# snudm-starlab/VMLMF

Hardware: AMD Instinct MI355X
Metric: RNN timesteps/sec (fwd+bwd) at B=64 T=128 hid=180 r=16; 1/2/4/8 GPU (higher is better)
Workload: dtype f32; 1 GPU; BASELINE configs[1]: UCI-HAR shape, Net(MyLSTM[MyVMLMFCell]) 1 layer, B=64/GPU T=128 I=9 H=180 w_rank=16 u_rank=16, CE loss, fwd+bwd; parameters packed inside every step, as a training loop sees it (with kept parameter images: ms_per_step_kept_images); global_batch=64, batch_per_gpu=64, seq_len=128, parallelism=dp1, scaling=weak, launch=hipgraph, parameter_images=packed inside every step (what a training loop sees), criterion=vmlmf_amd.Net.loss (cross-entropy riding on the forward launch, C ABI vmlmf_ce)

## Files before the change

vmlmf_amd/csrc/vmlmf_api.hip:

```cpp
#include "vmlmf_host.h"

using namespace vmlmf_host;

namespace vmlmf_host {

int make_geo(const vmlmf_desc* d, VGeo* out, RbGeo* rbout, int force_W) {
  if (d == nullptr) return fail(VMLMF_E_BADARG, "null descriptor");
  VGeo g;
  memset(&g, 0, sizeof(g));
  g.variant = d->variant;
  g.B = d->B;
  g.T = d->T;
  g.I = d->I;
  g.H = d->H;
  g.rw = d->w_rank;
  if (d->dtype != VMLMF_DT_F32 && d->dtype != VMLMF_DT_BF16) return fail(VMLMF_E_BADARG, "dtype must be VMLMF_DT_F32 or VMLMF_DT_BF16");
  g.bf = d->dtype == VMLMF_DT_BF16 ? 1 : 0;
  if (g.variant < 1 || g.variant > 6) return fail(VMLMF_E_BADARG, "variant must be 1..6");
  if (g.B < 1 || g.T < 1 || g.I < 1 || g.H < 1 || g.rw < 1)
    return fail(VMLMF_E_BADARG, "B, T, I, H, w_rank must be positive");
  const bool grouped = g.variant == VMLMF_V2_GROUP_CELL || g.variant == VMLMF_V4_LM_GROUP ||
                       g.variant == VMLMF_V6_GROUP_NOVM;
  const bool lm = g.variant == VMLMF_V3_LM || g.variant == VMLMF_V4_LM_GROUP;
  g.novm = (g.variant == VMLMF_V5_LMF_CELL || g.variant == VMLMF_V6_GROUP_NOVM) ? 1 : 0;
  g.pergate = g.variant == VMLMF_V5_LMF_CELL ? 1 : 0;
  g.xperm = g.variant == VMLMF_V6_GROUP_NOVM ? 1 : 0;
  g.G = grouped ? d->g : 1;
  if (grouped && g.G < 1) return fail(VMLMF_E_BADARG, "g must be positive");
  if (g.G > VMLMF_MAX_G)
    return fail(VMLMF_E_UNSUPPORTED, "g > 2 is not covered by the HIP kernels (the reference never builds it)");
  if (g.H % g.G != 0) return fail(VMLMF_E_SHAPE, "hidden_size must be divisible by g (vmlmf_group.py:73)");
  if (!lm && !g.novm && g.I > g.H)
    return fail(VMLMF_E_SHAPE, "input_size > hidden_size: the reference cell raises (vmlmf.py:94,103)");

  if (lm && g.I != g.H) return fail(VMLMF_E_SHAPE, "LM layers need input_size == hidden_size (vmlmf_lm.py:243)");
  g.ru0 = d->u_ranks[0];
  g.ru1 = g.G == 2 ? d->u_ranks[1] : 0;
  if (g.ru0 < 1 || (g.G == 2 && g.ru1 < 1)) return fail(VMLMF_E_BADARG, "u_ranks must be positive");
  g.Hg = g.H / g.G;
  g.W = (g.Hg + 63) / 64;
  if (force_W > g.W) g.W = force_W;
  g.NW = g.G * g.W;
  g.NT = g.NW * 64;
  g.off1 = vg_pad8(g.ru0);
  g.KH = g.off1 + (g.G == 2 ? vg_pad8(g.ru1) : 0);
  g.KX = vg_pad8(g.rw);
  g.NP = (g.KH + 15) / 16;
  g.KQ = g.NP * 16;
  g.NPX = (g.KX + 15) / 16;
  g.KQX = g.NPX * 16;
  g.flat = g.variant == VMLMF_V4_LM_GROUP ? 1 : 0;
  g.hperm = (g.variant == VMLMF_V2_GROUP_CELL || g.variant == VMLMF_V6_GROUP_NOVM) ? 1 : 0;
  g.time_major = d->time_major ? 1 : 0;
  g.training = d->training ? 1 : 0;
  if (g.time_major) {
    g.sxT = (long long)g.B * g.I;
    g.sxB = g.I;
    g.syT = (long long)g.B * g.H;
    g.syB = g.H;
  } else {
    g.sxT = g.I;
    g.sxB = (long long)g.T * g.I;
    g.syT = g.H;
    g.syB = (long long)g.T * g.H;
  }
  g.generic = (g.KH > 32 || g.NT > 512 || g.I > g.H) ? 1 : 0;
  g.wide = (g.KX > 32 || g.G * g.KH > 128) ? 1 : 0;
  if (g.wide) {
    if (!g.generic) {
      if (g.KX > 32)
        return fail(VMLMF_E_UNSUPPORTED, "padded w_rank > 32 is not covered by the HIP kernels on a register-resident layer "
                                         "(wide ranks need the step-wise path: padded u_rank > 32, more than 512 thread slots or I > H)");
      return fail(VMLMF_E_UNSUPPORTED, "padded hidden rank (summed over groups) > 128 is not covered on a register-resident layer");
    }
    if (g.rw > g.I) return fail(VMLMF_E_UNSUPPORTED, "wide ranks: w_rank larger than input_size (an over-complete factorisation) is not covered");
    if (g.ru0 > g.Hg || (g.G == 2 && g.ru1 > g.Hg))
      return fail(VMLMF_E_UNSUPPORTED, "wide ranks: a u_rank larger than the units it factors (hidden_size / g) is not covered");
    if (g.bf) return fail(VMLMF_E_UNSUPPORTED, "wide ranks: dtype bf16 is not covered (fp32 only)");
    if (g.KX > 1024 || g.KH > 1024)
      return fail(VMLMF_E_UNSUPPORTED, "wide ranks: padded w_rank and padded hidden rank (summed over shifts) are capped at 1024, the "
                                       "bound of the step-wise workspace");
  }
  g.R = 1;
  g.nwg = (g.B + g.R - 1) / g.R;
  g.Bp = g.nwg * g.R;
  if ((long long)g.T * g.Bp * g.NT * 4 >= (1LL << 31) || (long long)g.T * g.B * g.H >= (1LL << 31))
    return fail(VMLMF_E_UNSUPPORTED, "T*B*H too large for the 32-bit element offsets of the kernels");
  const int TB = g.T * g.B;
  int rc = ((TB + 1023) / 1024 + 7) / 8 * 8;
  if (rc < 8) rc = 8;
  if (g_rc > 0) rc = g_rc;
  g.RC = rc;
  g.nblk = (TB + rc - 1) / rc;
  int rc2 = (TB + g_wchunks - 1) / g_wchunks;
  if (rc2 < g_wmin) rc2 = g_wmin;
  g.RC2 = rc2;
  g.nchunk = (TB + rc2 - 1) / rc2;
  g.foldx = (!g.generic && g.I <= g.KX) ? 1 : 0;
  g.NA = 5 * g.KX + 5 * g.KH + 12;
  {
    RbGeo q;
    memset(&q, 0, sizeof(q));
    g.rb = 0;
    if (g.bf) {
      if (!g.generic && g.I <= g.H && rb_geometry(g, 1, &q, g_rb_rows)) g.rb = 1;
      else return fail(VMLMF_E_UNSUPPORTED, "dtype bf16: implemented by the row-block MFMA kernels for one-group layers (V1, V3, V5) "
                                            "with padded rank <= 32 and <= 512 thread slots");
    } else if (g_rb_mode != 0 && g.I <= g.H && !g.wide) {
      if (g.generic) {
        const int cand[] = {g_rb_S, 16, 8, 4, 2};
        for (int i = (g_rb_S > 0 ? 0 : 1); i < 5 && g.rb == 0; ++i)
          if (cand[i] > 1 && rb_geometry(g, cand[i], &q, g_rb_rows)) g.rb = cand[i];
      } else if ((g_rb_mode == 1 || (g_rb_minB > 0 && g.B >= g_rb_minB)) && rb_geometry(g, 1, &q, g_rb_rows)) {
        g.rb = 1;
      }
    }
    if (g.rb != 0) g.foldx = 0;
    if (rbout != nullptr) *rbout = q;
  }
  {
    const long long GK = (long long)g.G * g.KH;
    const long long nb1 = (vg_nb1(g) + 31) / 32 * 32, nb2 = (GK + 31) / 32 * 32, nb3 = (g.KX + 31) / 32 * 32;
    g.PCH = (long long)g.NT * 4 * nb1 + (long long)((g.H + 31) / 32) * 32 * nb2 +
            (long long)((g.I + 31) / 32) * 32 * nb3 + 3LL * g.NT * 4;
  }
  *out = g;
  return 0;
}

static long long gemm_part_floats(const VGeo& g) { return (long long)VG_GEMM_SPLIT * ((g.B + 63) / 64 * 64) * ((g.G * g.KH + 63) / 64 * 64); }
Layout make_layout(const VGeo& g, const VPack& P, const RbGeo& q) {
  Layout L;
  const long long TB = (long long)g.T * g.B;
  const long long TS = (long long)g.T * g.Bp * g.NT;
  long long o = 0;
  L.r_pack = o, o += align64(P.total);
  const long long TBp = TB + (g.NT >= 256 ? 16 : 0);
  L.r_qx = o, o += align64(TBp * g.KX);
  L.r_gates = o, o += align64(TS * 4);
  L.r_cs = o, o += align64(TS + (long long)g.Bp * g.NT);
  L.r_Qs = o, o += align64(TBp * g.G * g.KH);
  L.r_prog = o, o += align64((long long)g.B * WR_PROG_STRIDE);
  L.r_total = o;
  o = 0;
  L.f_pack = o, o += align64(P.total);
  L.f_gx = o, o += align64(TS * 4);
  L.f_qx = o, o += align64(g.generic ? TB * g.KX : 0);
  L.f_trash = o, o += 64;
  {
    const long long gen = (g.generic && !g.rb) ? 1 : 0, BN = (long long)g.B * g.NT;
    L.f_Qtmp = o, o += align64(gen * g.B * g.G * g.KH);
    L.f_P = o, o += align64(gen * BN * 4);
    L.f_ccar = o, o += align64(gen * BN);
    L.f_zeros = o, o += align64(gen * (long long)g.B * g.H);
    L.f_part = o, o += align64(gen * gemm_part_floats(g));
  }
  L.f_xq = o, o += align64(g.rb ? q.xq_floats : 0);
  L.f_flag = o, o += align64(g.rb ? q.flag_words : 0);
  L.f_xrows = o, o += align64((g.wide && !g.time_major) ? TB * g.I : 0);
  L.f_total = o;
  o = 0;
  L.b_dpre = o, o += align64(TS * 4);
  L.b_dQs = o, o += align64(TBp * g.G * g.KH);
  L.b_dqx = o, o += align64(TBp * g.KX);
  {
    long long blocks = g.nchunk;
    if (!g.generic && !g.rb && rec4_bwd_supported(g) && g.nwg > blocks) blocks = g.nwg;
    L.b_wpart = o, o += align64(g.wide ? 0 : blocks * g.PCH);
  }
  L.b_cgrad = o, o += align64((long long)g.NA * g.NT + (g.I > g.H ? (long long)g.I * g.KX : 0));
  L.b_trash = o, o += 64;
  {
    const long long gen = (g.generic && !g.rb) ? 1 : 0, BN = (long long)g.B * g.NT;
    L.b_dHrec = o, o += align64(gen * (long long)g.B * g.H);
    L.b_ehterm = o, o += align64(gen * BN);
    L.b_dcar = o, o += align64(gen * BN);
    L.b_part = o, o += align64((g.generic ? 1 : 0) * gemm_part_floats(g));
  }
  L.b_xq = o, o += align64(g.rb ? q.xq_floats : 0);
  L.b_flag = o, o += align64(g.rb ? q.flag_words : 0);
  L.b_headdh = o, o += align64((g.rb || g.generic) ? (long long)g.B * g.H : 0);
  L.b_dux = o, o += align64((!g.generic && !g.rb && finish2_ok(g)) ? (long long)g.nchunk * (g.NT / 8) * 256 : 0);
  L.b_wide = o, o += wide_scratch_floats(g);
  L.b_total = o;
  return L;
}

template <class P>
static int check_pointers(const VGeo& g, const P* p, const char* what) {
  if (p == nullptr) return fail(VMLMF_E_BADARG, std::string("null ") + what);
  bool ok = p->u_x && p->u_h[0];
  if (g.pergate) {
    for (int k = 0; k < 4; ++k) ok = ok && p->w_gate[k] && p->u_gate[k] && p->b_gate[k];
  } else {
    ok = ok && p->v_x && p->b_x && p->b_h && p->v_h[0];
    if (!g.novm) ok = ok && p->dia_x && p->dia_h;
  }
  if (!ok) return fail(VMLMF_E_BADARG, std::string("null pointer in ") + what);
  if (g.G == 2 && (!p->u_h[1] || !p->v_h[1]))
    return fail(VMLMF_E_BADARG, std::string(what) + ": group variant needs u_h[1], v_h[1]");
  return 0;
}

int check_params(const VGeo& g, const vmlmf_params* p) { return check_pointers(g, p, "params"); }
int check_grads(const VGeo& g, const vmlmf_grads* gr) { return check_pointers(g, gr, "grads"); }
int check_head(const VGeo& g, const vmlmf_head* hd, bool fwd) {
  if (hd == nullptr || hd->classes == 0) return 0;
  if (hd->classes < 0 || hd->classes > head_max_classes()) return fail(VMLMF_E_UNSUPPORTED, "head: 1..32 classes");
  if (hd->weight == nullptr || (fwd ? hd->logits == nullptr : hd->dlogits == nullptr)) return fail(VMLMF_E_BADARG, "head: null pointer");
  return 0;
}

static void plan_wride(const VGeo& g, WRide* w) {
  const int n1 = (vg_nb1(g) + 31) / 32, n2 = (g.G * g.KH + 31) / 32;
  if (!g_wride || g_wride_tripped.load() != 0 || !g.foldx || g.flat || g.R != 1 || g.NT > 256 || g.B > g_wride_maxb || n1 > 2 || n2 > 2) return;
  const int S = (g.B % g_wride_rc == 0 && g_wride_rc % 2 == 0) ? g_wride_rc : g.B * (g.B >= 64 ? 1 : (64 + g.B - 1) / g.B);
  const int nck = (g.T * g.B + S - 1) / S;
  int K = g_wride_k < g.nchunk ? g_wride_k : g.nchunk;
  K = K < nck ? K : nck;
  const int tasks = g.NT / 8 + (g.H + 31) / 32;
  const int wpw = (g.NT + 128) / 64;
  const int ntg = (tasks + wpw - 1) / wpw;
  const int room = (device_cus() - 8 - g.nwg) / ntg;
  K = K < room ? K : room;
  if (K < 4) return;
  w->K = K, w->S = S, w->tasks = tasks, w->ntg = ntg;
  w->lag = g_wride_lag < 8 ? g_wride_lag : 8;
  w->spin = (unsigned)g_wride_spin;
}

LayerPlan plan_layer(const VGeo& g, const vmlmf_params* p, bool packed, bool head, bool want_dx, PlanCtx ctx) {
  LayerPlan pl;
  memset(&pl, 0, sizeof(pl));
  pl.family = g.rb ? FAM_RB : (g.generic ? FAM_STEP : FAM_VALU);
  pl.xwave = g_xwave && vg_xwave_ok(g);
  pl.head_inside = head && pl.family == FAM_VALU;
  pl.dqx = !(g.foldx && !want_dx);
  if (pl.family != FAM_VALU) return pl;
  const bool call = ctx == PLAN_CALL;
  if (pl.xwave && ((g_rec3 & 1) || ((g_rec3 & 4) && g.nwg > device_cus())) && rec3_fwd_supported(g)) pl.fwd = K_REC3;
  const bool rec3_bwd = (g_rec3 & 2) && rec3_bwd_supported(g);
  if (call && g_inrow != 0 && !want_dx && rec4_bwd_supported(g) && (g_inrow > 0 || g.B > g_wride_maxb)) pl.bwd = K_REC4;
  else pl.bwd = rec3_bwd ? K_REC3 : K_REC;
  if (call && pl.bwd != K_REC4) plan_wride(g, &pl.ride);
  if (pl.ride.K > 0 && pl.bwd != K_REC3 && !rec_bwd_rides(g)) memset(&pl.ride, 0, sizeof(pl.ride));
  pl.finish2 = pl.ride.K > 0 && g_finish2 != 0 && finish2_ok(g) && p->v_x != nullptr;
  const uintptr_t al = (uintptr_t)p->v_h[0] | (uintptr_t)p->u_h[0] | (uintptr_t)p->v_x | (uintptr_t)p->u_x;
  pl.direct = call && !packed && g_direct != 0 && (g.variant == VMLMF_V1_CELL || g.variant == VMLMF_V3_LM) && g.G == 1 && g.R == 1 &&
              g.foldx && pl.xwave && pl.fwd == K_REC && (g.KH == 8 || g.KH == 16) && g.ru0 == g.KH && (g.KX == 8 || g.KX == 16) &&
              g.rw == g.KX && (!g.training || rec3_bwd) && (al & 15u) == 0;
  return pl;
}

static WgxArgs wgx_args(const Layout& L, const VPack& P, const float* pack, float* ws, float* dx) {
  WgxArgs wx;
  wx.dpre = ws + L.b_dpre, wx.VRX = pack + P.VRX, wx.UXO = pack + P.UXO, wx.EXI = pack + P.EXI;
  wx.dx = dx, wx.dqx = ws + L.b_dqx;
  return wx;
}
static void split_k(GenericBuf* w, const VGeo& g, float* part, const float* pack, const VPack& P) {
  w->part = part, w->part_cap = gemm_part_floats(g);
  w->ticket = reinterpret_cast<int*>(const_cast<float*>(pack + P.TKT)), w->ticket_cap = VG_GEMM_TICKETS;
}
static void ride_buffers(LayerPlan* pl, const Layout& L, const WghArgs& wh, const vmlmf_params* p, const float* rs, float* ws, hipStream_t s) {
  WRide* w = &pl->ride;
  if (pl->bwd == K_REC4) {
    w->a.x = wh.x, w->a.y = wh.y, w->a.h0 = wh.h0, w->a.Qs = wh.Qs, w->a.P = wh.wpart;
    return;
  }
  if (w->K == 0) return;
  w->a.dpre = wh.dpre, w->a.x = wh.x, w->a.y = wh.y, w->a.h0 = wh.h0, w->a.qx = wh.qx, w->a.dqx = wh.dqx, w->a.Qs = wh.Qs;
  w->a.dQs = wh.dQs, w->a.P = wh.wpart;
  w->prog = reinterpret_cast<unsigned*>(const_cast<float*>(rs + L.r_prog));
  w->status = status_word(s);
  if (pl->finish2) w->dux = ws + L.b_dux, w->vx = p->v_x;
}

int backward_tail(const VGeo& g, const LayerPlan& pl, const Layout& L, const vmlmf_params* p, const vmlmf_grads* gr, const float* x,
                  const float* y, const float* h0, const float* rs, float* ws, const HeadBwd& hb, hipStream_t s) {
  int rc;
  const WghArgs wh = wgrad_args(L, x, y, h0, rs, ws);
  const bool rode = pl.ride.K > 0, inrow = pl.bwd == K_REC4;
  int ring_nc[3] = {0, 0, 0};
  if (g.wide) {
    const long long TB = (long long)g.T * g.B, N4 = 4LL * g.NT, GK = (long long)g.G * g.KH;
    auto al = [](long long n) { return (n + 63) / 64 * 64; };
    WideBuf wb;
    wb.x = x, wb.y = y, wb.h0 = h0, wb.dpre = wh.dpre, wb.qx = wh.qx, wb.dqx = wh.dqx, wb.Qs = wh.Qs, wb.dQs = wh.dQs;
    float* o = ws + L.b_wide;
    wb.X = o, o += al(g.time_major ? 0 : TB * g.I);
    wb.Hp = o, o += al(TB * g.H);
    wb.dVd = o, o += al(N4 * GK);
    wb.dUd = o, o += al((long long)g.H * GK);
    wb.dVx = o, o += al(N4 * g.KX);
    wb.dUx = o, o += al((long long)g.I * g.KX);
    wb.csum = o;
    wb.cgrad = ws + L.b_cgrad;
    if ((rc = run(SL_WGRAD, s, "wgrad", [&] { return wide_wgrad(g, wb, s); })) != 0) return rc;
  } else if (!rode && !inrow) {
    Scope sc(SL_WGRAD, s);
    const bool ring = g_wring != 0 && wgrad_ring_ok(g) && (g_wring > 0 || (g.generic && (long long)g.T * g.B >= 1024));
    int rr = ring ? launch_wgrad_ring(g, wh, device_cus(), ring_nc, s) : -3;
    if (rr == 0) ++g_ring_launches;
    if (rr == -3) {
      ring_nc[0] = ring_nc[1] = ring_nc[2] = 0;
      rr = launch_wgrad_h(g, wh, s);
    }
    if ((rc = hip_fail(rr, "wgrad")) != 0) return rc;
  }
  const RefG og = to_refg(gr);
  if (rode && pl.finish2)
    return run(SL_FINISH2, s, "finish2", [&] {
      return launch_finish2(g, to_refp(p), ws + L.b_wpart, pl.ride.dux, pl.ride.K, og, hb, pl.ride.prog, s, health_word(s));
    });
  if (!g.wide) {
    VGeo gr_ = g;
    if (rode) gr_.nchunk = pl.ride.K;
    if (inrow) gr_.nchunk = g.B;
    if ((rc = run(SL_REDUCE, s, "reduce", [&] {
           return launch_reduce(gr_, ws + L.b_wpart, ws + L.b_cgrad, rode ? pl.ride.prog : nullptr, s, ReduceCounts{{ring_nc[0], ring_nc[1], ring_nc[2]}});
         })) != 0) return rc;
  }
  return run(SL_FINISH, s, "finish", [&] { return launch_finish(g, to_refp(p), ws + L.b_cgrad, og, hb, s, health_word(s)); });
}

int site_drop(const vmlmf_dropout* dr, bool forward, DropArgs* out) {
  memset(out, 0, sizeof(*out));
  if (dr == nullptr) return 0;
  const int rc = drop_args(dr->p, dr->state, dr->site, forward ? dr->y_dropped : nullptr, out);
  if (rc != 0) return rc;
  if (dr->state == nullptr || (forward && dr->y_dropped == nullptr)) return fail(VMLMF_E_BADARG, "dropout: null state / y_dropped");
  return 0;
}

int valu_backward(const VGeo& g, LayerPlan* pl, const Layout& L, const VPack& P, const float* pack, const vmlmf_params* p, const LayerBwdIo& io,
                  const HeadBwd& hb, const float* rs, float* ws, hipStream_t s) {
  int rc;
  BwdArgs a;
  a.gates = rs + L.r_gates, a.cs = rs + L.r_cs, a.c0 = io.c0, a.dy = io.dy, a.dhT = io.dhT, a.dcT = io.dcT;
  a.VR = pack + P.VR, a.UE = pack + P.UE, a.EH = pack + P.EH, a.VE = pack + P.VE;
  a.dpre = ws + L.b_dpre, a.dQs = ws + L.b_dQs, a.dh0 = io.dh0, a.dc0 = io.dc0, a.trash = ws + L.b_trash;
  a.hd = hb;
  ride_buffers(pl, L, wgrad_args(L, io.x, io.y, io.h0, rs, ws), p, rs, ws, s);
  a.wr = pl->ride;
  if (pl->direct) {
    const bool own = pl->bwd == K_REC4 || pl->ride.K > 0;
    if (own) a.VE = p->v_h[0], a.UE = p->u_h[0], a.EH = p->dia_h, a.wr.direct = 1;
    if ((!own || pl->dqx) &&
        (rc = run(SL_PACK, s, "pack", [&] { return launch_pack(g, to_refp(p), P, const_cast<float*>(pack), s); })) != 0) return rc;
  }
  {
    Scope sc(SL_REC_BWD, s);
    if (pl->bwd == K_REC4) {
      if ((rc = hip_fail(launch_rec4_bwd(g, a, s), "rec4_bwd")) != 0) return rc;
    } else if (pl->bwd == K_REC3) {
      if ((rc = hip_fail(launch_rec3_bwd(g, a, s), "rec3_bwd")) != 0) return rc;
    } else if ((rc = hip_fail(launch_rec_bwd(g, a, s), "rec_bwd")) != 0) return rc;
  }
  if (!pl->dqx) return 0;
  return run(SL_DQX_DX, s, "dqx_dx", [&] { return launch_wgrad_x(g, wgx_args(L, P, pack, ws, io.dx), s); });
}

}

extern "C" {

int vmlmf_query(const vmlmf_desc* d, vmlmf_sizes* out) {
  if (out == nullptr) return fail(VMLMF_E_BADARG, "null sizes");
  VGeo g;
  RbGeo q;
  const int rc = make_geo(d, &g, &q);
  if (rc != 0) return rc;
  const VPack P = vg_pack_layout(g, q.total);
  const Layout L = make_layout(g, P, q);
  out->workspace_bytes = (size_t)L.ws_total() * sizeof(float);
  out->reserve_bytes = (size_t)L.r_total * sizeof(float);
  out->rows_per_wg = g.rb ? q.rbl : g.R;
  out->threads_per_wg = g.rb ? 256 : g.NT;
  out->workgroups = g.rb ? q.nrb * q.S : g.nwg;
  out->kx = g.KX;
  out->kh = g.KH;
  return 0;
}

constexpr int PK_HDR = 64;
struct PackSig {
  long long v[10];
  bool operator==(const PackSig& o) const { return memcmp(v, o.v, sizeof(v)) == 0; }
};
static PackSig pack_signature(const VGeo& g, const VPack& P, const RbGeo& q) {
  PackSig s;
  const long long v[10] = {g.variant, P.total, g.rb, g.generic * 2 + g.bf, g.NT, (long long)g.KH * 1000 + g.KX, q.total,
                           (long long)g.I * 100000 + g.H, (long long)g.G * 100000 + g.ru0 * 100 + g.ru1, g_tune_generation};
  memcpy(s.v, v, sizeof(v));
  return s;
}
constexpr int PK_REG = 256;
struct PackReg {
  std::mutex mu;
  const void* ptr[PK_REG] = {nullptr};
  PackSig sig[PK_REG];
  int next = 0;
  void put(const void* p, const PackSig& s) {
    std::lock_guard<std::mutex> lk(mu);
    for (int i = 0; i < PK_REG; ++i)
      if (ptr[i] == p) { sig[i] = s; return; }
    ptr[next] = p, sig[next] = s;
    next = (next + 1) % PK_REG;
  }
  int check(const void* p, const PackSig& s) {
    std::lock_guard<std::mutex> lk(mu);
    for (int i = 0; i < PK_REG; ++i)
      if (ptr[i] == p) return sig[i] == s ? 0 : 2;
    return 1;
  }
} g_packreg;
static int refuse_kept(const char* why = "") {
  return fail(VMLMF_E_UNSUPPORTED, std::string("kept parameter images: not for the step-wise / clustered layers") + why);
}
static int check_packed(const void* packed, const VGeo& g, const VPack& P, const RbGeo& q) {
  if (g.generic) return refuse_kept();
  switch (g_packreg.check(packed, pack_signature(g, P, q))) {
    case 0: return 0;
    case 1: return fail(VMLMF_E_BADARG, "packed: not an image vmlmf_pack_params made at this address (or it left the registry of the last 256 images: pack it again)");
  }
  return fail(VMLMF_E_BADARG, "packed: the image was packed for another descriptor or under another kernel selection (vmlmf_tune): pack it again");
}

int vmlmf_pack_bytes(const vmlmf_desc* d, size_t* bytes) {
  if (bytes == nullptr) return fail(VMLMF_E_BADARG, "null size");
  VGeo g;
  RbGeo q;
  const int rc = make_geo(d, &g, &q);
  if (rc != 0) return rc;
  if (g.generic) return refuse_kept(" (their image carries per-call state)");
  const VPack P = vg_pack_layout(g, q.total);
  *bytes = sizeof(float) * (size_t)(PK_HDR + P.total);
  return 0;
}

int vmlmf_pack_params(const vmlmf_desc* d, const vmlmf_params* p, void* packed, void* stream) {
  VGeo g;
  RbGeo q;
  int rc = make_geo(d, &g, &q);
  if (rc != 0) return rc;
  if ((rc = check_params(g, p)) != 0) return rc;
  if (packed == nullptr) return fail(VMLMF_E_BADARG, "null packed buffer");
  if (g.generic) return refuse_kept();
  const VPack P = vg_pack_layout(g, q.total);
  hipStream_t s = (hipStream_t)stream;
  float* img = (float*)packed + PK_HDR;
  g_packreg.put(packed, pack_signature(g, P, q));
  const RefP rp = to_refp(p);
  Scope sc(SL_PACK, s);
  if ((rc = hip_fail(launch_pack(g, rp, P, img, s), "pack")) != 0) return rc;
  if (g.rb && (rc = hip_fail(launch_rb_pack(g, q, rp, img + P.RB, s), "rb_pack")) != 0) return rc;
  return 0;
}

int vmlmf_seq_forward(const vmlmf_desc* d, const vmlmf_params* p, const float* x, const float* h0,
                      const float* c0, float* y, float* hT, float* cT, void* reserve, void* workspace,
                      size_t workspace_bytes, void* stream) {
  return vmlmf_seq_forward_packed(d, p, x, h0, c0, y, hT, cT, reserve, workspace, workspace_bytes, stream, nullptr);
}

int vmlmf_seq_forward_packed(const vmlmf_desc* d, const vmlmf_params* p, const float* x, const float* h0,
                             const float* c0, float* y, float* hT, float* cT, void* reserve, void* workspace,
                             size_t workspace_bytes, void* stream, const void* packed) {
  vmlmf_extra ex = {};
  ex.packed = packed, ex.head = nullptr, ex.ce = nullptr;
  return vmlmf_seq_forward_ex(d, p, x, h0, c0, y, hT, cT, reserve, workspace, workspace_bytes, stream, &ex);
}

static int ce_after(int B, const vmlmf_head* head, const vmlmf_ce* ce, hipStream_t s) {
  if (ce == nullptr) return 0;
  return run(SL_CE_FWD, s, "ce_fwd", [&] {
    return launch_ce_fwd(B, head->classes, head->logits, (const long long*)ce->target, (long long)ce->ignore_index, ce->loss, ce->lse,
                         ce->nvalid, ce->dlogits_unit, s);
  });
}
static int head_and_ce_after(const VGeo& g, const vmlmf_head* head, const vmlmf_ce* ce, const float* hT, hipStream_t s) {
  int rc;
  if (head != nullptr && (rc = run(SL_HEAD_FWD, s, "head_fwd", [&] {
        return launch_head_fwd(g.B, g.H, head->classes, hT, g.H, head->weight, head->bias, head->logits, s);
      })) != 0) return rc;
  return ce_after(g.B, head, ce, s);
}

static int make_drop(const vmlmf_dropout* dr, const VGeo& g, bool forward, DropArgs* out) {
  const int rc = site_drop(dr, forward, out);
  if (rc != 0 || dr == nullptr || drop_fused(g)) return rc;
  return fail(VMLMF_E_UNSUPPORTED, "dropout inside the layer's launches: row-block layers in the time-major layout (vmlmf_dropout_fused)");
}

int vmlmf_seq_forward_ex(const vmlmf_desc* d, const vmlmf_params* p, const float* x, const float* h0,
                         const float* c0, float* y, float* hT, float* cT, void* reserve, void* workspace,
                         size_t workspace_bytes, void* stream, const vmlmf_extra* ex) {
  const void* packed = ex != nullptr ? ex->packed : nullptr;
  const vmlmf_head* head = (ex != nullptr && ex->head != nullptr && ex->head->classes != 0) ? ex->head : nullptr;
  VGeo g;
  RbGeo q;
  int rc = take_status();
  if (rc != 0) return rc;
  if ((rc = make_geo(d, &g, &q)) != 0) return rc;
  if ((rc = check_params(g, p)) != 0) return rc;
  if (x == nullptr || y == nullptr || workspace == nullptr) return fail(VMLMF_E_BADARG, "null x / y / workspace");
  if (g.training && reserve == nullptr) return fail(VMLMF_E_BADARG, "training forward needs a reserve buffer");
  if ((rc = check_head(g, head, true)) != 0) return rc;
  const LayerPlan pl = plan_layer(g, p, packed != nullptr, head != nullptr, true);
  if (head != nullptr && !pl.head_inside && hT == nullptr) return fail(VMLMF_E_BADARG, "head on this layer needs the hT output");
  DropArgs drop;
  if ((rc = make_drop(ex != nullptr ? ex->drop : nullptr, g, true, &drop)) != 0) return rc;
  const vmlmf_ce* ce = ex != nullptr ? ex->ce : nullptr;
  if (ce != nullptr) {
    if (head == nullptr) return fail(VMLMF_E_BADARG, "ce: the criterion rides on the classifier's logits (extra.head)");
    if (!ce->target || !ce->loss || !ce->nvalid || !ce->lse || !ce->ticket) return fail(VMLMF_E_BADARG, "ce: null pointer");
  }
  const VPack P = vg_pack_layout(g, q.total);
  const Layout L = make_layout(g, P, q);
  if (workspace_bytes < (size_t)L.ws_total() * sizeof(float))
    return fail(VMLMF_E_WORKSPACE, "workspace smaller than vmlmf_query() reported");
  hipStream_t s = (hipStream_t)stream;
  float* ws = (float*)workspace;
  float* rs = (float*)reserve;
  float* pack = g.training ? rs + L.r_pack : ws + L.f_pack;
  if (packed != nullptr) {
    if ((rc = check_packed(packed, g, P, q)) != 0) return rc;
    pack = const_cast<float*>((const float*)packed) + PK_HDR;
  }
  float* gx = ws + L.f_gx;
  const RefP rp = to_refp(p);
  if (packed == nullptr && !pl.direct && (rc = run(SL_PACK, s, "pack", [&] { return launch_pack(g, rp, P, pack, s); })) != 0) return rc;
  float* const qxbuf = g.training ? rs + L.r_qx : (g.generic ? ws + L.f_qx : nullptr);
  if (!pl.xwave && (rc = run(SL_XPROJ, s, "xproj", [&] {
        return g.wide ? wide_xproj(g, P, pack, x, ws + L.f_xrows, gx, qxbuf, s) : launch_xproj(g, P, pack, x, gx, qxbuf, s);
      })) != 0) return rc;
  if (pl.family == FAM_RB) {
    if (packed == nullptr && (rc = run(SL_PACK, s, "rb_pack", [&] {
          return launch_rb_pack(g, q, rp, pack + P.RB, s, reinterpret_cast<unsigned*>(ws + L.f_flag));
        })) != 0) return rc;
    RbIo io;
    memset(&io, 0, sizeof(io));
    io.flags_zeroed = packed == nullptr ? 1 : 0;
    io.gx = gx, io.EH = pack + P.EH, io.h0 = h0, io.c0 = c0, io.img = pack + P.RB, io.y = y, io.hT = hT, io.cT = cT;
    io.gates = g.training ? rs + L.r_gates : nullptr, io.cs = g.training ? rs + L.r_cs : nullptr;
    io.Qs = g.training ? rs + L.r_Qs : nullptr;
    io.xq = ws + L.f_xq, io.flag = reinterpret_cast<unsigned*>(ws + L.f_flag), io.status = status_word(s);
    io.drop = drop;
    if ((rc = run(SL_REC_FWD, s, "rb_fwd", [&] { return launch_rb_fwd(g, q, io, s); })) != 0) return rc;
    return head_and_ce_after(g, head, ce, hT, s);
  }
  if (pl.family == FAM_STEP) {
    GenericBuf w;
    memset(&w, 0, sizeof(w));
    w.gx = gx, w.EH = pack + P.EH, w.h0 = h0, w.c0 = c0, w.Ud = pack + P.UD, w.Vd = pack + P.VD;
    w.UdT = pack + P.UDT;
    w.zeros = ws + L.f_zeros, w.y = y, w.hT = hT, w.cT = cT;
    w.gates = g.training ? rs + L.r_gates : nullptr, w.cs = g.training ? rs + L.r_cs : nullptr;
    w.Qs = g.training ? rs + L.r_Qs : nullptr, w.Qtmp = ws + L.f_Qtmp, w.P = ws + L.f_P, w.ccar = ws + L.f_ccar;
    split_k(&w, g, ws + L.f_part, pack, P);
    if (h0 == nullptr) {
      rc = (int)hipMemsetAsync(ws + L.f_zeros, 0, sizeof(float) * (size_t)g.B * g.H, s);
      if (rc != 0) return hip_fail(rc, "memset");
    }
    if ((rc = run(SL_REC_FWD, s, "generic_forward", [&] { return generic_forward(g, w, s); })) != 0) return rc;
    return head_and_ce_after(g, head, ce, hT, s);
  }
  FwdArgs a;
  a.gx = gx, a.VE = pack + P.VE, a.UR = pack + P.UR, a.EH = pack + P.EH, a.h0 = h0, a.c0 = c0;
  a.y = y, a.hT = hT, a.cT = cT, a.trash = ws + L.f_trash;
  a.gates = g.training ? rs + L.r_gates : nullptr;
  a.cs = g.training ? rs + L.r_cs : nullptr;
  a.Qs = g.training ? rs + L.r_Qs : nullptr;
  XwArgs xw;
  xw.x = x, xw.UXP = pack + P.UXP, xw.WXD = pack + P.WXD, xw.BBT = pack + P.BBT;
  memset(&xw.hd, 0, sizeof(xw.hd));
  if (pl.head_inside) xw.hd.W = head->weight, xw.hd.bias = head->bias, xw.hd.logits = head->logits, xw.hd.C = head->classes;
  memset(&xw.ce, 0, sizeof(xw.ce));
  if (pl.head_inside && ce != nullptr && g.R == 1 && g.B < 65536) {
    xw.ce.tgt = (const long long*)ce->target, xw.ce.ignore = (long long)ce->ignore_index, xw.ce.loss = ce->loss, xw.ce.nvalid = ce->nvalid;
    xw.ce.lse = ce->lse, xw.ce.dz = ce->dlogits_unit, xw.ce.ticket = (unsigned long long*)ce->ticket;
  }
  a.xwave = pl.xwave ? 1 : 0, a.qxw = g.training ? rs + L.r_qx : nullptr;
  xw.BH = nullptr, xw.DX = nullptr, xw.direct = 0, xw.pad = 0;
  if (pl.direct) {
    a.VE = p->v_h[0], a.UR = p->u_h[0], a.EH = p->dia_h, a.xwave = 3;
    xw.UXP = p->u_x, xw.WXD = p->v_x, xw.BBT = p->b_x, xw.BH = p->b_h, xw.DX = p->dia_x, xw.direct = 1;
  }
  a.prog = g.training ? reinterpret_cast<unsigned*>(rs + L.r_prog) : nullptr;
  if ((rc = pl.fwd == K_REC3 ? run(SL_REC_FWD, s, "rec3_fwd", [&] { return launch_rec3_fwd(g, a, xw, s); })
                             : run(SL_REC_FWD, s, "rec_fwd", [&] { return launch_rec_fwd(g, a, xw, s); })) != 0) return rc;
  if (ce != nullptr && xw.ce.tgt == nullptr && (rc = ce_after(g.B, head, ce, s)) != 0) return rc;
  return debug_status(s);
}

int vmlmf_seq_backward(const vmlmf_desc* d, const vmlmf_params* p, const float* x, const float* h0,
                       const float* c0, const float* y, const void* reserve, const float* dy,
                       const float* dhT, const float* dcT, float* dx, float* dh0, float* dc0,
                       const vmlmf_grads* gr, void* workspace, size_t workspace_bytes, void* stream) {
  return vmlmf_seq_backward_packed(d, p, x, h0, c0, y, reserve, dy, dhT, dcT, dx, dh0, dc0, gr, workspace, workspace_bytes, stream,
                                   nullptr);
}

int vmlmf_seq_backward_packed(const vmlmf_desc* d, const vmlmf_params* p, const float* x, const float* h0,
                              const float* c0, const float* y, const void* reserve, const float* dy,
                              const float* dhT, const float* dcT, float* dx, float* dh0, float* dc0,
                              const vmlmf_grads* gr, void* workspace, size_t workspace_bytes, void* stream,
                              const void* packed) {
  vmlmf_extra ex = {};
  ex.packed = packed, ex.head = nullptr, ex.ce = nullptr;
  return vmlmf_seq_backward_ex(d, p, x, h0, c0, y, reserve, dy, dhT, dcT, dx, dh0, dc0, gr, workspace, workspace_bytes, stream, &ex);
}

int vmlmf_seq_backward_ex(const vmlmf_desc* d, const vmlmf_params* p, const float* x, const float* h0,
                          const float* c0, const float* y, const void* reserve, const float* dy,
                          const float* dhT, const float* dcT, float* dx, float* dh0, float* dc0,
                          const vmlmf_grads* gr, void* workspace, size_t workspace_bytes, void* stream,
                          const vmlmf_extra* ex) {
  const void* packed = ex != nullptr ? ex->packed : nullptr;
  const vmlmf_head* head = (ex != nullptr && ex->head != nullptr && ex->head->classes != 0) ? ex->head : nullptr;
  VGeo g;
  RbGeo q;
  int rc = take_status();
  if (rc != 0) return rc;
  if ((rc = make_geo(d, &g, &q)) != 0) return rc;
  if ((rc = check_params(g, p)) != 0) return rc;
  if (x == nullptr || y == nullptr || reserve == nullptr || workspace == nullptr || gr == nullptr)
    return fail(VMLMF_E_BADARG, "null x / y / reserve / workspace / grads");
  if ((rc = check_grads(g, gr)) != 0) return rc;
  if ((rc = check_head(g, head, false)) != 0) return rc;
  LayerPlan pl = plan_layer(g, p, packed != nullptr, head != nullptr, dx != nullptr);
  DropArgs drop;
  if ((rc = make_drop(ex != nullptr ? ex->drop : nullptr, g, false, &drop)) != 0) return rc;
  const VPack P = vg_pack_layout(g, q.total);
  const Layout L = make_layout(g, P, q);
  if (workspace_bytes < (size_t)L.ws_total() * sizeof(float))
    return fail(VMLMF_E_WORKSPACE, "workspace smaller than vmlmf_query() reported");
  hipStream_t s = (hipStream_t)stream;
  float* ws = (float*)workspace;
  const float* rs = (const float*)reserve;
  const float* hlast = y + (size_t)(g.T - 1) * g.syT;
  const HeadBwd hb = head_bwd_args(pl.head_inside ? head : nullptr, g, y);
  if (head != nullptr && !pl.head_inside) {
    if (dhT != nullptr) return fail(VMLMF_E_UNSUPPORTED, "head together with an explicit dhT: only on the VALU recurrent kernels");
    float* tmp = ws + L.b_headdh;
    if ((rc = run(SL_HEAD_BWD, s, "head_bwd", [&] {
           return launch_head_bwd(g.B, g.H, head->classes, hlast, g.syB, head->weight, head->dlogits, tmp, head->dweight, head->dbias, s);
         })) != 0) return rc;
    dhT = tmp;
  }
  const float* pack = rs + L.r_pack;
  if (packed != nullptr) {
    if ((rc = check_packed(packed, g, P, q)) != 0) return rc;
    pack = (const float*)packed + PK_HDR;
  }
  if (pl.family == FAM_RB) {
    RbIo io;
    memset(&io, 0, sizeof(io));
    io.gates = const_cast<float*>(rs + L.r_gates), io.cs = const_cast<float*>(rs + L.r_cs), io.EH = pack + P.EH;
    io.img = pack + P.RB, io.dy = dy, io.dhT = dhT, io.dcT = dcT, io.dpre = ws + L.b_dpre, io.dQs = ws + L.b_dQs;
    io.dh0 = dh0, io.dc0 = dc0, io.xq = ws + L.b_xq, io.flag = reinterpret_cast<unsigned*>(ws + L.b_flag), io.status = status_word(s);
    io.drop = drop;
    if ((rc = run(SL_REC_BWD, s, "rb_bwd", [&] { return launch_rb_bwd(g, q, io, s); })) != 0) return rc;
    if (g.generic) {
      GenericBuf w;
      memset(&w, 0, sizeof(w));
      w.dpre = ws + L.b_dpre, w.VxT = pack + P.VXTT, w.dqx = ws + L.b_dqx, w.dx = dx, w.UXP = pack + P.UXP, w.EXT = pack + P.EXT;
      split_k(&w, g, ws + L.b_part, pack, P);
      if ((rc = run(SL_DQX_DX, s, "dqx_dx", [&] { return generic_dqx_dx(g, w, s); })) != 0) return rc;
    } else if ((rc = run(SL_DQX_DX, s, "dqx_dx", [&] { return launch_wgrad_x(g, wgx_args(L, P, pack, ws, dx), s); })) != 0) {
      return rc;
    }
  } else if (pl.family == FAM_STEP) {
    GenericBuf w;
    memset(&w, 0, sizeof(w));
    w.EH = pack + P.EH, w.gates = const_cast<float*>(rs + L.r_gates), w.cs = const_cast<float*>(rs + L.r_cs);
    w.dy = dy, w.dhT = dhT, w.dcT = dcT, w.UdT = pack + P.UDT, w.VdT = pack + P.VDT, w.VxT = pack + P.VXTT;
    w.UXP = pack + P.UXP, w.EXT = pack + P.EXT, w.Vd = pack + P.VD;
    w.dpre = ws + L.b_dpre, w.dQs = ws + L.b_dQs, w.dHrec = ws + L.b_dHrec, w.ehterm = ws + L.b_ehterm;
    w.dcar = ws + L.b_dcar, w.dh0 = dh0, w.dc0 = dc0, w.dqx = ws + L.b_dqx, w.dx = dx;
    if (g.wide) {
      w.UXT = pack + P.UXT;
      w.dxs = ws + L.b_total - ((long long)g.T * g.B * g.I + 63) / 64 * 64;
    }
    split_k(&w, g, ws + L.b_part, pack, P);
    if ((rc = run(SL_REC_BWD, s, "generic_backward", [&] { return generic_backward(g, w, s); })) != 0) return rc;
  } else if ((rc = valu_backward(g, &pl, L, P, pack, p, LayerBwdIo{x, y, h0, c0, dy, dhT, dcT, dx, dh0, dc0}, hb, rs, ws, s)) != 0) {
    return rc;
  }
  if ((rc = backward_tail(g, pl, L, p, gr, x, y, h0, rs, ws, hb, s)) != 0) return rc;
  return debug_status(s);
}

}
```

vmlmf_amd/csrc/vmlmf_host.h:

```cpp
#pragma once
#include <hip/hip_runtime.h>

#include <atomic>
#include <cstdio>
#include <cstring>
#include <mutex>
#include <string>
#include <vector>

#include "../../include/vmlmf_hip.h"
#include "vmlmf_launch.h"

#pragma GCC visibility push(hidden)
namespace vmlmf_host {

int fail(int code, const std::string& msg);
int hip_fail(int rc, const char* what);
inline int hip_tail(int rc) { return rc == 0 ? 0 : fail(rc, hipGetErrorString((hipError_t)rc)); }

extern int g_debug_sync, g_adam_guard, g_xwave, g_wchunks, g_wmin, g_rc, g_wride, g_wride_k, g_wride_maxb, g_wride_lag, g_wride_rc, g_rb_mode,
    g_rb_minB, g_rb_S, g_rb_rows, g_rec3, g_inrow, g_wring, g_direct, g_finish2, g_wf_bwd, g_pack_slim, g_finish_units, g_rbx, g_ffb;
extern int g_wride_spin, g_tune_generation;
extern std::atomic<int> g_wride_tripped;
extern std::atomic<int> g_ring_launches;

enum Slot { SL_PACK, SL_XPROJ, SL_REC_FWD, SL_REC_BWD, SL_DQX_DX, SL_WGRAD, SL_REDUCE, SL_FINISH, SL_HEAD_FWD, SL_HEAD_BWD, SL_CE_FWD,
            SL_CE_BWD, SL_FINISH2, NKERN };
inline const char* kernel_label(int k) {
  static const char* const names[NKERN] = {"pack_kernel",     "xproj_kernel",      "rec_fwd_kernel",   "rec_bwd_kernel",
                                           "dqx_dx_kernel",   "wgrad_mfma_kernel", "reduce_cg_kernel", "finish_kernel",
                                           "head_fwd_kernel", "head_bwd_kernel",   "ce_fwd_kernel",    "ce_bwd_kernel", "finish2_kernel"};
  return (k >= 0 && k < NKERN) ? names[k] : "";
}
struct Prof {
  std::mutex mu;
  unsigned mask = 0;
  std::vector<std::pair<hipEvent_t, hipEvent_t>> ev[NKERN];
};
extern Prof g_prof;

struct Scope {
  int k;
  hipStream_t s;
  hipEvent_t e0 = nullptr, e1 = nullptr;
  Scope(Slot which, hipStream_t st) : k(which), s(st) {
    if (g_debug_sync) fprintf(stderr, "[vmlmf] launching %s\n", kernel_label(which));
    if ((g_prof.mask >> which) & 1u) {
      (void)hipEventCreate(&e0);
      (void)hipEventCreate(&e1);
      (void)hipEventRecord(e0, s);
    }
  }
  ~Scope() {
    if (g_debug_sync) {
      const hipError_t e = hipStreamSynchronize(s);
      fprintf(stderr, "[vmlmf] %s done: %s\n", kernel_label(k), hipGetErrorString(e));
    }
    if (e0 != nullptr) {
      (void)hipEventRecord(e1, s);
      std::lock_guard<std::mutex> lk(g_prof.mu);
      g_prof.ev[k].push_back({e0, e1});
    }
  }
};
template <class F>
int run(Slot k, hipStream_t s, const char* what, F&& launch) {
  Scope sc(k, s);
  return hip_fail((int)launch(), what);
}

unsigned* status_word(hipStream_t s);
unsigned* health_word(hipStream_t s);
int take_status();
int debug_status(hipStream_t s);
int device_cus();

inline long long align64(long long v) { return (v + 63) / 64 * 64; }
int make_geo(const vmlmf_desc* d, VGeo* out, RbGeo* rbout = nullptr, int force_W = 0);
struct Layout {
  long long r_pack, r_qx, r_gates, r_cs, r_Qs, r_prog, r_total;
  long long f_pack, f_gx, f_qx, f_trash, f_Qtmp, f_P, f_ccar, f_zeros, f_part, f_xq, f_flag, f_xrows, f_total;
  long long b_dpre, b_dQs, b_dqx, b_wpart, b_cgrad, b_trash, b_dHrec, b_ehterm, b_dcar, b_part, b_xq, b_flag, b_headdh, b_dux, b_wide, b_total;
  long long ws_total() const { return f_total > b_total ? f_total : b_total; }
};
Layout make_layout(const VGeo& g, const VPack& P, const RbGeo& q);

inline RefP to_refp(const vmlmf_params* p) {
  RefP r;
  r.dia_x = p->dia_x, r.dia_h = p->dia_h, r.u_x = p->u_x, r.v_x = p->v_x, r.b_x = p->b_x, r.b_h = p->b_h;
  r.u_h0 = p->u_h[0], r.u_h1 = p->u_h[1], r.v_h0 = p->v_h[0], r.v_h1 = p->v_h[1];
  for (int k = 0; k < 4; ++k) r.wg[k] = p->w_gate[k], r.ug[k] = p->u_gate[k], r.bg[k] = p->b_gate[k];
  return r;
}
inline RefG to_refg(const vmlmf_grads* gr) {
  RefG og;
  og.dia_x = gr->dia_x, og.dia_h = gr->dia_h, og.u_x = gr->u_x, og.v_x = gr->v_x, og.b_x = gr->b_x;
  og.b_h = gr->b_h, og.u_h0 = gr->u_h[0], og.u_h1 = gr->u_h[1], og.v_h0 = gr->v_h[0], og.v_h1 = gr->v_h[1];
  for (int k = 0; k < 4; ++k) og.wg[k] = gr->w_gate[k], og.ug[k] = gr->u_gate[k], og.bg[k] = gr->b_gate[k];
  return og;
}

int check_params(const VGeo& g, const vmlmf_params* p);
int check_grads(const VGeo& g, const vmlmf_grads* gr);
int check_head(const VGeo& g, const vmlmf_head* hd, bool fwd);

inline int drop_args(float p, const void* state, int site, float* yd, DropArgs* out) {
  memset(out, 0, sizeof(*out));
  if (!(p >= 0.f && p < 1.f)) return fail(VMLMF_E_BADARG, "dropout: p must be in [0, 1)");
  out->state = reinterpret_cast<const unsigned long long*>(state), out->yd = yd;
  out->thresh = drop_thresh(p), out->scale = 1.f / (1.f - p), out->site = site;
  return 0;
}
int site_drop(const vmlmf_dropout* dr, bool forward, DropArgs* out);
inline bool drop_fused(const VGeo& g) { return g.rb && g.syT == (long long)g.B * g.H; }

enum Family { FAM_RB, FAM_STEP, FAM_VALU };
enum RecKernel { K_REC, K_REC3, K_REC4 };
enum PlanCtx { PLAN_CALL, PLAN_CHAINED };
struct LayerPlan {
  Family family;
  bool xwave;
  RecKernel fwd, bwd;
  bool direct;
  bool head_inside;
  bool dqx;
  bool finish2;
  WRide ride;
};
LayerPlan plan_layer(const VGeo& g, const vmlmf_params* p, bool packed, bool head, bool want_dx, PlanCtx ctx = PLAN_CALL);

inline WghArgs wgrad_args(const Layout& L, const float* x, const float* y, const float* h0, const float* rs, float* ws) {
  WghArgs wh;
  wh.dpre = ws + L.b_dpre, wh.x = x, wh.y = y, wh.h0 = h0, wh.qx = rs + L.r_qx, wh.dqx = ws + L.b_dqx;
  wh.Qs = rs + L.r_Qs, wh.dQs = ws + L.b_dQs, wh.wpart = ws + L.b_wpart;
  return wh;
}
inline HeadBwd head_bwd_args(const vmlmf_head* head, const VGeo& g, const float* y) {
  HeadBwd hb;
  memset(&hb, 0, sizeof(hb));
  if (head == nullptr) return hb;
  hb.W = head->weight, hb.dl = head->dlogits, hb.hlast = y + (size_t)(g.T - 1) * g.syT, hb.ldh = g.syB, hb.dW = head->dweight, hb.db = head->dbias;
  hb.C = head->classes;
  return hb;
}
struct LayerBwdIo {
  const float *x, *y, *h0, *c0, *dy, *dhT, *dcT;
  float *dx, *dh0, *dc0;
};
int valu_backward(const VGeo& g, LayerPlan* pl, const Layout& L, const VPack& P, const float* pack, const vmlmf_params* p, const LayerBwdIo& io,
                  const HeadBwd& hb, const float* rs, float* ws, hipStream_t s);
int backward_tail(const VGeo& g, const LayerPlan& pl, const Layout& L, const vmlmf_params* p, const vmlmf_grads* gr, const float* x,
                  const float* y, const float* h0, const float* rs, float* ws, const HeadBwd& hb, hipStream_t s);

}
#pragma GCC visibility pop
```

vmlmf_amd/csrc/vmlmf_launch.h:

```cpp
#pragma once
#include <hip/hip_runtime.h>
#include "vmlmf_device.h"
#include "vmlmf_dropout.h"

#define VG_REC_BOUNDS (MAXT + 128)

enum EnvRule { ENV_SET, ENV_ON, ENV_INT, ENV_POS };
int vmlmf_env_switch(const char* name, EnvRule rule, int dflt);

struct HeadFwd {
  const float *W, *bias;
  float* logits;
  int C, pad;
};
struct HeadBwd {
  const float *W, *dl;
  const float* hlast;
  float *dW, *db;
  long long ldh;
  int C, pad;
};

struct FwdArgs {
  const float *gx, *VE, *UR, *EH, *h0, *c0;
  float *y, *hT, *cT, *gates, *cs, *Qs;
  float* trash;
  float* qxw;
  int xwave;
  unsigned* prog;
};
struct CeFwd {
  const long long* tgt;
  long long ignore;
  float *loss, *nvalid;
  float *lse, *dz;
  unsigned long long* ticket;
};
struct XwArgs {
  const float *x, *UXP, *WXD, *BBT;
  HeadFwd hd;
  CeFwd ce;
  const float *BH, *DX;
  int direct, pad;
};
struct AtbArgs {
  const float *dpre, *x, *y, *h0, *qx, *dqx, *Qs, *dQs;
  float* P;
  int pad0, pad;
};
constexpr int WR_PROG_STRIDE = 32;
constexpr unsigned VMLMF_ST_WRIDE = 1, VMLMF_ST_CLUSTER = 2, VMLMF_ST_WF_FWD = 3, VMLMF_ST_WF_BWD = 4, VMLMF_ST_P2P = 5;
__device__ __forceinline__ void vg_raise(unsigned* status, unsigned code) {
  if (status != nullptr) __hip_atomic_store(status, code, __ATOMIC_RELAXED, __HIP_MEMORY_SCOPE_SYSTEM);
}
struct WRide {
  AtbArgs a;
  float* dux;
  const float* vx;
  unsigned* prog;
  int K, S, ntg, tasks;
  int lag;
  int direct;
  unsigned spin;
  unsigned* status;
};
struct BwdArgs {
  const float *gates, *cs, *c0, *dy, *dhT, *dcT, *VR, *UE, *EH;
  const float* VE;
  float *dpre, *dQs, *dh0, *dc0;
  float* trash;
  HeadBwd hd;
  WRide wr;
};
struct WgxArgs {
  const float *dpre, *VRX, *UXO, *EXI;
  float *dx, *dqx;
};
struct WghArgs {
  const float *dpre, *x, *y, *h0, *qx, *dqx, *Qs, *dQs;
  float* wpart;
};

struct GenericBuf {
  const float *gx, *EH, *h0, *c0, *Ud, *Vd, *zeros;
  float *y, *hT, *cT, *gates, *cs, *Qs, *Qtmp, *P, *ccar;
  const float *dy, *dhT, *dcT, *UdT, *VdT, *VxT, *UXP, *EXT;
  float *dpre, *dQs, *dHrec, *ehterm, *dcar, *dh0, *dc0, *dqx, *dx;
  const float* UXT;
  float* dxs;
  float* part;
  long long part_cap;
  int* ticket;
  int ticket_cap;
};
int generic_forward(const VGeo& g, const GenericBuf& w, hipStream_t s);
int generic_backward(const VGeo& g, const GenericBuf& w, hipStream_t s);
int generic_dqx_dx(const VGeo& g, const GenericBuf& w, hipStream_t s);
int generic_qx(const VGeo& g, const float* x, const float* UXP, float* qx, hipStream_t s);
int wide_xproj(const VGeo& g, const VPack& L, const float* pack, const float* x, float* xrows, float* gx, float* qx, hipStream_t s);
constexpr int WIDE_NCH = 64;
struct WideBuf {
  const float *x, *y, *h0, *dpre, *qx, *dqx, *Qs, *dQs;
  float *X, *Hp;
  float *dVd, *dUd, *dVx, *dUx;
  float *csum;
  float *cgrad;
};
inline long long wide_scratch_floats(const VGeo& g) {
  if (!g.wide) return 0;
  const long long TB = (long long)g.T * g.B, N4 = 4LL * g.NT, GK = (long long)g.G * g.KH;
  auto al = [](long long n) { return (n + 63) / 64 * 64; };
  return al(g.time_major ? 0 : TB * g.I) + al(TB * g.H) + al(N4 * GK) + al((long long)g.H * GK) + al(N4 * g.KX) +
         al((long long)g.I * g.KX) + al((long long)WIDE_NCH * 3 * N4) + al(TB * g.I);
}
int wide_wgrad(const VGeo& g, const WideBuf& w, hipStream_t s);

constexpr int RBX_MAXL = 4;
struct RbIo {
  const float *gx, *EH, *h0, *c0, *img, *dy, *dhT, *dcT;
  float *y, *hT, *cT, *gates, *cs, *Qs, *dpre, *dQs, *dh0, *dc0;
  float* xq;
  unsigned* flag;
  unsigned* status;
  int flags_zeroed;
  DropArgs drop;
};
bool rb_geometry(const VGeo& g, int S, RbGeo* out, int rows = 0, int xf = 0);

struct RbxLayerF {
  const float *x, *EH, *EXT, *BBT, *h0, *c0, *img;
  float *y, *hT, *cT, *gates, *cs, *Qs, *qx;
  float* xq;
  unsigned* flag;
  const unsigned* pflag;
  int pub, pad;
  DropArgs drop;
};
struct RbxLayerB {
  const float *gates, *cs, *dy, *dhT, *dcT, *EH, *EXT, *img;
  float *dpre, *dQs, *dqx, *dx, *dh0, *dc0;
  float* xq;
  unsigned* flag;
  const unsigned* pflag;
  int pub, pad;
  DropArgs drop;
};
struct RbxFwdArgs {
  unsigned* status;
  int L, bpl;
  RbxLayerF l[RBX_MAXL];
};
struct RbxBwdArgs {
  unsigned* status;
  int L, bpl;
  RbxLayerB l[RBX_MAXL];
};
struct RbxZeroArgs {
  float* dpre[RBX_MAXL];
  unsigned* flags[RBX_MAXL];
};
bool rbx_supported(const VGeo& g, const RbGeo& q);
int launch_rbx_fwd(const VGeo& g, const RbGeo& q, const RbxFwdArgs& a, hipStream_t s);
int launch_rbx_bwd(const VGeo& g, const RbGeo& q, const RbxBwdArgs& a, hipStream_t s);
int launch_rbx_zero(const VGeo& g, const RbGeo& q, int L, float* const* dpre, unsigned* const* flags, hipStream_t s);
int launch_rb_pack(const VGeo& g, const RbGeo& q, const RefP& p, float* img, hipStream_t s, unsigned* zero_flags = nullptr);
int launch_rb_fwd(const VGeo& g, const RbGeo& q, const RbIo& io, hipStream_t s);
int launch_rb_pack_stack(const VGeo& g, const RbGeo& q, int L, const RefP* p, float* const* img, unsigned* const* zero_flags, hipStream_t s);
int launch_rb_bwd(const VGeo& g, const RbGeo& q, const RbIo& io, hipStream_t s);

int launch_pack(const VGeo& g, const RefP& p, const VPack& L, float* pack, hipStream_t s);
int launch_xproj(const VGeo& g, const VPack& L, const float* pack, const float* x, float* gx, float* qx,
                 hipStream_t s);
int launch_rec_fwd(const VGeo& g, const FwdArgs& a, const XwArgs& xw, hipStream_t s);
int launch_rec_bwd(const VGeo& g, const BwdArgs& a, hipStream_t s);
inline bool rec_bwd_rides(const VGeo& g) { return g.KH > 16 || g.W > 3; }
bool rec3_fwd_supported(const VGeo& g);
bool rec3_bwd_supported(const VGeo& g);
int launch_rec3_fwd(const VGeo& g, const FwdArgs& a, const XwArgs& xw, hipStream_t s);
int launch_rec3_bwd(const VGeo& g, const BwdArgs& a, hipStream_t s);
bool rec4_bwd_supported(const VGeo& g);
int launch_rec4_bwd(const VGeo& g, const BwdArgs& a, hipStream_t s);
int launch_wgrad_x(const VGeo& g, const WgxArgs& a, hipStream_t s);
int launch_wgrad_h(const VGeo& g, const WghArgs& a, hipStream_t s);
bool wgrad_ring_ok(const VGeo& g);
int launch_wgrad_ring(const VGeo& g, const WghArgs& a, int cus, int nc_out[3], hipStream_t s);
struct ReduceCounts {
  int c[3];
};
int launch_reduce(const VGeo& g, const float* wpart, float* cgrad, unsigned* prog, hipStream_t s,
                  ReduceCounts wc = ReduceCounts{{0, 0, 0}});
bool finish2_ok(const VGeo& g);
int launch_finish2(const VGeo& g, const RefP& p, const float* wpart, const float* dux, int K, const RefG& out, const HeadBwd& hd,
                   unsigned* prog, hipStream_t s, unsigned* health);
int launch_finish(const VGeo& g, const RefP& p, const float* cgrad, const RefG& out, const HeadBwd& hd, hipStream_t s,
                  unsigned* health = nullptr);
unsigned* vmlmf_health_word_if_any();
int vmlmf_adam_guard_mode();

int head_max_classes();
hipError_t launch_head_fwd(int B, int H, int C, const float* h, long long ldh, const float* W, const float* bias,
                           float* out, hipStream_t s);
hipError_t launch_head_bwd(int B, int H, int C, const float* h, long long ldh, const float* W, const float* dl,
                           float* dh, float* dW, float* db, hipStream_t s);

hipError_t launch_ce_fwd(int B, int C, const float* z, const long long* tgt, long long ignore_index, float* loss,
                         float* lse, float* nvalid, float* dz_unit, hipStream_t s);
hipError_t launch_ce_bwd(int B, int C, const float* z, const long long* tgt, long long ignore_index,
                         const float* lse, const float* nvalid, const float* dloss, float* dz, hipStream_t s);

hipError_t launch_nll_fwd(int R, int V, const float* scores, const long long* y, float scale, float* loss, float* lse,
                          float* rowloss, hipStream_t s);
hipError_t launch_nll_bwd(int R, int V, const float* scores, const long long* y, float scale, const float* lse,
                          const float* dloss, float* dscores, hipStream_t s);

int head_loss_workgroups(int R);
int launch_nll_fwd_grad(int R, int V, float* scores, const float* bias, const long long* y, float scale, float* loss,
                        float* rowloss, float* dbias, float* scratch, hipStream_t s);
int launch_distill_fwd_grad(int R, int V, float* scores, const float* bias, const long long* y, float scale, float alpha, float tau,
                            const float* teacher, const long long* top_tokens, const float* top_scores, int top, float* loss,
                            float* rowloss, float* dbias, float* scratch, hipStream_t s);
struct ObjectiveArgs {
  float eps, zeta, alpha;
  const long long* negatives;
  int k;
  const float* scale_dev;
};
int launch_objective_fwd_grad(int R, int V, float* scores, const float* bias, const long long* y, float scale, const ObjectiveArgs& o,
                              float* loss, float* rowloss, float* dbias, float* scratch, hipStream_t s);
size_t embed_bwd_scratch_bytes(int R, int V);
int launch_transpose(int rows, int cols, const float* src, float* dst, hipStream_t s);
int launch_embed_bwd(int R, int H, int V, const long long* tokens, const float* dy, float* dW, void* scratch, size_t scratch_bytes,
                     hipStream_t s, const DropArgs* drop = nullptr);
int launch_drop_advance(unsigned long long* state, unsigned long long* snap, hipStream_t s);
int launch_drop_rows(int mode, long long R, int H, int V, const DropArgs& d, const DropCols& cm, const float* x, const long long* tokens, float* y,
                     hipStream_t s);
struct LmSampleArgs {
  const float *h, *w, *bias, *embed;
  const unsigned long long* state;
  long long* tokens;
  float *logprob, *x_next;
  float* part;
  unsigned long long* ticket;
  float inv_temp;
  int B, H, V, step, tpw;
  int top_k;
  float top_p;
  int* kept;
  float* scores;
};
size_t lm_sample_workspace_bytes(int B, int V);
size_t lm_sample_filtered_workspace_bytes(int B, int V);
int launch_lm_sample(LmSampleArgs a, hipStream_t s);
struct LmChooseArgs {
  const float *scores, *bias, *embed;
  const unsigned long long* state;
  long long* tokens;
  float *logprob, *x_next;
  float inv_temp;
  int B, H, V, step;
  int top_k;
  float top_p;
  int* kept;
};
int launch_lm_choose(const LmChooseArgs& a, hipStream_t s);

constexpr int WF_MAXL = 4;
constexpr int WF_FLAG_STRIDE = 32;
struct WfPack {
  long long UR, VR, URX, VRX;
  long long VE, UE, VXK, UXK;
  long long total;
};
__host__ __device__ inline int wf_width(const VGeo& g) { return g.KH > g.KX ? g.KH : g.KX; }
struct WfFwdLayer {
  const float* x;
  const float *VE, *EH, *VXT, *EXT, *BBT;
  const float *UR, *URX;
  const float *h0, *c0;
  float *y, *hT, *cT, *gates, *cs, *Qs, *qx;
  long long sxT, sxB;
  long long syT, syB;
  int I, H;
  int Hg, pad;
};
struct WfBwdLayer {
  const float *gates, *cs, *dy, *dhT, *dcT;
  const float *UE, *EH, *UXO, *EXI;
  const float *VR, *VRX;
  float *dpre, *dQs, *dqx, *dx, *dh0, *dc0;
  long long sxT, sxB;
  long long syT, syB;
  int I, want_dx;
  int H, Hg;
};
struct WfCommon {
  unsigned* flag;
  unsigned* status;
  int L, pad;
};
struct WfFwdArgs {
  WfCommon c;
  WfFwdLayer l[WF_MAXL];
  HeadFwd hd;
  DropArgs drop[WF_MAXL];
};
struct WfBwdArgs {
  WfCommon c;
  WfBwdLayer l[WF_MAXL];
  HeadBwd hd;
  DropArgs drop[WF_MAXL];
};
bool wf_supported(const VGeo& g);
WfPack wf_pack_layout(const VGeo& g);
int launch_pack_stack(int L, const VGeo* g, const RefP* p, const VPack* P, const WfPack& W, float* const* pack, unsigned* zero0,
                      int nzero0, unsigned* zero1, int nzero1, hipStream_t s, int images = 0);
enum { PACK_ALL = 0, PACK_CLUSTERED = 1, PACK_WAVEFRONT = 2 };
int launch_wf_fwd(const VGeo& g, const WfFwdArgs& a, hipStream_t s);
int launch_wf_bwd(const VGeo& g, const WfBwdArgs& a, hipStream_t s);
int launch_wgrad_h_stack(int L, const VGeo* g, const WghArgs* w, hipStream_t s);
struct AtbStack;
int launch_wgrad4_stack(int L, const VGeo* g, const WghArgs* w, const AtbStack& S, hipStream_t s);
int wgrad4_chunk_rows(int L, const VGeo* g, int cus);
int launch_reduce_stack(int L, const VGeo* g, const float* const* wpart, float* const* cgrad, hipStream_t s,
                        const ReduceCounts* wc = nullptr);
bool finish_from_blocks_ok(const VGeo& g);
int launch_finish_stack(int L, const VGeo* g, const RefP* p, const float* const* cgrad, const RefG* out, const HeadBwd& hd_top,
                        hipStream_t s, unsigned* health = nullptr, const float* const* wpart = nullptr,
                        const ReduceCounts* wc = nullptr);
bool finish_units_ok(const VGeo& g);
int launch_finish_units_stack(int L, const VGeo* g, const RefP* p, const RefG* out, const HeadBwd& hd_top, hipStream_t s,
                              unsigned* health, const float* const* wpart, const ReduceCounts* wc);

bool rec_supported(const VGeo& g);
```

vmlmf_amd/csrc/vmlmf_rec_fwd.inc:

```
#include "vmlmf_launch.h"
#include "vmlmf_direct.inc"

constexpr int FWD_NB = 6;


template <typename S>
__device__ __forceinline__ void copy_from_kernarg(S* dst, const __attribute__((address_space(4))) char* src) {
  static_assert(sizeof(S) % 4 == 0, "dword-sized argument structs");
  const __attribute__((address_space(4))) int* w = (const __attribute__((address_space(4))) int*)src;
  int tmp[sizeof(S) / 4];
#pragma unroll
  for (unsigned i = 0; i < sizeof(S) / 4; ++i) tmp[i] = w[i];
  __builtin_memcpy(dst, tmp, sizeof(S));
}
constexpr size_t karg_align8(size_t v) { return (v + 7) & ~(size_t)7; }
constexpr size_t KARG_FWD = karg_align8(sizeof(VGeo));
constexpr size_t KARG_XW = karg_align8(KARG_FWD + sizeof(FwdArgs));

__device__ __forceinline__ float wave_total(float v) {
  v = add_ror16<8>(v);
  v = add_ror16<4>(v);
  v = add_ror16<2>(v);
  v = add_ror16<1>(v);
  return rowsum4(v);
}
__device__ __forceinline__ float wave_max64(float v) {
#pragma unroll
  for (int o = 32; o >= 1; o >>= 1) v = fmaxf(v, __shfl_xor(v, o, 64));
  return v;
}
__device__ __attribute__((noinline)) void head_epilogue(const __attribute__((address_space(4))) char* ka,
                                                        const __attribute__((address_space(3))) float* ch, int row, int wave,
                                                        __attribute__((address_space(3))) float* lscr) {
  if (((const __attribute__((address_space(4))) int*)(ka + KARG_XW + offsetof(XwArgs, hd) + offsetof(HeadFwd, C)))[0] <= 0) return;
  VGeo g;
  XwArgs xa;
  copy_from_kernarg(&g, ka);
  copy_from_kernarg(&xa, ka + KARG_XW);
  const HeadFwd hd = xa.hd;
  if (hd.C <= 0 || row >= g.B) return;
  const int lane = threadIdx.x & 63, H = g.H, NT = g.NT, C = hd.C, NW = g.NW;
  constexpr int CP = 8;
  for (int c0 = wave; c0 < C; c0 += CP * NW) {
    float acc[CP];
#pragma unroll
    for (int j = 0; j < CP; ++j) acc[j] = 0.f;
    for (int slot = lane; slot < NT; slot += 64) {
      int n;
      const bool valid = vg_slot_unit(g, slot, n);
      const float hv = valid ? ch[slot * 2 + 1] : 0.f;
      const int nc = valid ? n : 0;
      float w[CP];
#pragma unroll
      for (int j = 0; j < CP; ++j) w[j] = hd.W[(size_t)(c0 + j * NW < C ? c0 + j * NW : 0) * H + nc];
#pragma unroll
      for (int j = 0; j < CP; ++j) acc[j] = fmaf(hv, c0 + j * NW < C ? w[j] : 0.f, acc[j]);
    }
#pragma unroll
    for (int j = 0; j < CP; ++j) {
      const float t = wave_total(acc[j]);
      const int c = c0 + j * NW;
      if (lane == 0 && c < C) {
        const float z = t + (hd.bias != nullptr ? hd.bias[c] : 0.f);
        hd.logits[(size_t)row * C + c] = z;
        lscr[c] = z;
      }
    }
  }
}

__device__ __attribute__((noinline)) void ce_epilogue(const __attribute__((address_space(4))) char* ka, int row, int wave,
                                                      __attribute__((address_space(3))) float* lscr) {
  if (((const __attribute__((address_space(4))) long long*)(ka + KARG_XW + offsetof(XwArgs, ce) + offsetof(CeFwd, tgt)))[0] == 0) return;
  VGeo g;
  XwArgs xa;
  copy_from_kernarg(&g, ka);
  copy_from_kernarg(&xa, ka + KARG_XW);
  const CeFwd ce = xa.ce;
  const int lane = threadIdx.x & 63, C = xa.hd.C, B = g.B;
  if (C <= 0 || row >= B) return;
  asm volatile("s_waitcnt lgkmcnt(0)\n\ts_barrier" ::: "memory");
  if (wave != 0) return;
  const float z = lane < C ? lscr[lane] : -INFINITY;
  const float m = wave_max64(z);
  const float l = m + logf(wave_total(lane < C ? expf(z - m) : 0.f));
  int cnt = 0;
  for (int b = lane; b < B; b += 64) cnt += ce.tgt[b] != ce.ignore ? 1 : 0;
#pragma unroll
  for (int o = 32; o >= 1; o >>= 1) cnt += __shfl_xor(cnt, o, 64);
  const float nv = (float)cnt, scale = 1.f / nv;
  const long long t = ce.tgt[row];
  const bool counted = t != ce.ignore, inr = t >= 0 && t < C;
  const float rl = counted ? (inr ? l - lscr[inr ? (int)t : 0] : NAN) : 0.f;
  if (ce.dz != nullptr && lane < C) ce.dz[(size_t)row * C + lane] = counted ? scale * (expf(z - l) - (lane == (int)t ? 1.f : 0.f)) : 0.f;
  typedef unsigned long long u64;
  int lb = 0;
  while ((1 << lb) < B) ++lb;
  const int SH = 35 - lb;
  const bool fits = rl >= 0.f && rl < 2048.f;
  u64 mine = (u64)1 << 48, old = 0;
  if (fits) mine += (u64)__double2ll_rn((double)rl * (double)((u64)1 << SH));
  if (lane == 0) {
    ce.lse[row] = l;
    if (!fits) {
      const bool nan = rl != rl, big = !nan && !(rl < (float)((u64)1 << (36 - lb)));
      const u64 add1 = nan ? (u64)1 << 63 : (big ? (u64)1 << 62 : (u64)__double2ll_rn((double)rl * 1024.0));
      u64 r1;
      if (nan || big) r1 = __hip_atomic_fetch_or(ce.ticket + 1, add1, __ATOMIC_RELAXED, __HIP_MEMORY_SCOPE_AGENT);
      else r1 = __hip_atomic_fetch_add(ce.ticket + 1, add1, __ATOMIC_RELAXED, __HIP_MEMORY_SCOPE_AGENT);
      asm volatile("" :: "v"(r1) : "memory");
      __hip_atomic_fetch_or(ce.ticket, (u64)1 << 47, __ATOMIC_RELAXED, __HIP_MEMORY_SCOPE_AGENT);
    }
    old = __hip_atomic_fetch_add(ce.ticket, mine, __ATOMIC_RELAXED, __HIP_MEMORY_SCOPE_AGENT);
  }
  const unsigned olo = __builtin_amdgcn_readfirstlane((unsigned)old), ohi = __builtin_amdgcn_readfirstlane((unsigned)(old >> 32));
  const u64 total = (((u64)ohi << 32) | olo) + mine, flag = total & ((u64)1 << 47);
  if ((unsigned)(total >> 48) != (unsigned)B) return;
  double sum = (double)(total & (((u64)1 << 47) - 1)) / (double)((u64)1 << SH);
  if (flag != 0) {
    const u64 w1 = __hip_atomic_load(ce.ticket + 1, __ATOMIC_RELAXED, __HIP_MEMORY_SCOPE_AGENT);
    sum += (double)(w1 & (((u64)1 << 47) - 1)) / 1024.0;
    if ((w1 >> 62) & 1) sum = (double)INFINITY;
    if ((w1 >> 63) & 1) sum = (double)NAN;
  }
  if (lane == 0) {
    ce.loss[0] = (float)(sum / (double)nv);
    ce.nvalid[0] = nv;
    __hip_atomic_store(ce.ticket, (u64)0, __ATOMIC_RELAXED, __HIP_MEMORY_SCOPE_AGENT);
    if (flag != 0) __hip_atomic_store(ce.ticket + 1, (u64)0, __ATOMIC_RELAXED, __HIP_MEMORY_SCOPE_AGENT);
  }
}

constexpr int XW_SLOTS = 3;
constexpr int XW_NB = 12;
constexpr int XW_DIST = 8;

__host__ __device__ inline size_t xwave_lds_floats() { return (size_t)XW_NB * 64 + 2 * 32; }

template <int IM, int IE = IM>
__device__ __attribute__((noinline)) void xwave_role(const __attribute__((address_space(4))) char* ka, float* gxs,
                                                     float* xlds, int row, int ring_nb) {
  VGeo g;
  XwArgs xa;
  copy_from_kernarg(&g, ka);
  copy_from_kernarg(&xa, ka + KARG_XW);
  const int lane = threadIdx.x & 63;
  const int I = g.I, H = g.H, NT = g.NT, T = g.T, KX = g.KX;
  typedef __attribute__((address_space(3))) float lds_f;
  typedef __attribute__((address_space(3))) f32x4 lds_f4;
  lds_f* xring = (lds_f*)xlds;
  lds_f* qxs = xring + XW_NB * 64;
  lds_f* gxl = (lds_f*)gxs;
  const bool rowok = row < g.B;
  const int rowc = rowok ? row : g.B - 1;

  f32x2 w01[XW_SLOTS][IM], w23[XW_SLOTS][IM], b01[XW_SLOTS], b23[XW_SLOTS];
  float uxc[IM];
  bool real[XW_SLOTS];
  if (xa.direct != 0) {
    asm volatile("s_waitcnt lgkmcnt(0)\n\ts_barrier" ::: "memory");
    const lds_f* wxl = (const lds_f*)xlds + xwave_lds_floats();
#pragma unroll
    for (int i = 0; i < XW_SLOTS; ++i) {
      const int slot = lane + 64 * i;
      real[i] = slot < NT;
      const int sc = real[i] ? slot : 0;
#pragma unroll
      for (int m = 0; m < IM; ++m) {
        const bool mk = real[i] && m < I;
        const int mc = m < I ? m : 0;
        const float q0 = wxl[(mc * 4 + 0) * NT + sc], q1 = wxl[(mc * 4 + 1) * NT + sc];
        const float q2 = wxl[(mc * 4 + 2) * NT + sc], q3 = wxl[(mc * 4 + 3) * NT + sc];
        w01[i][m] = mk ? f32x2{q0, q1} : f32x2{0.f, 0.f};
        w23[i][m] = mk ? f32x2{q2, q3} : f32x2{0.f, 0.f};
      }
      const float c0 = wxl[(4 * I + 0) * NT + sc], c1 = wxl[(4 * I + 1) * NT + sc], c2 = wxl[(4 * I + 2) * NT + sc], c3 = wxl[(4 * I + 3) * NT + sc];
      b01[i] = real[i] ? f32x2{c0, c1} : f32x2{0.f, 0.f};
      b23[i] = real[i] ? f32x2{c2, c3} : f32x2{0.f, 0.f};
    }
  } else
#pragma unroll
  for (int i = 0; i < XW_SLOTS; ++i) {
    const int slot = lane + 64 * i;
    int n = 0;
    real[i] = slot < NT;
    const bool valid = real[i] && vg_slot_unit(g, slot, n);
    const int sc = real[i] ? slot : 0, nc = valid ? n : 0;
#pragma unroll
    for (int m = 0; m < IM; ++m) {
      const bool mk = valid && m < I;
      const int mc = m < I ? m : 0;
      w01[i][m] = mk ? f32x2{xa.WXD[(size_t)(mc * 4 + 0) * NT + sc], xa.WXD[(size_t)(mc * 4 + 1) * NT + sc]} : f32x2{0.f, 0.f};
      w23[i][m] = mk ? f32x2{xa.WXD[(size_t)(mc * 4 + 2) * NT + sc], xa.WXD[(size_t)(mc * 4 + 3) * NT + sc]} : f32x2{0.f, 0.f};
    }
    b01[i] = valid ? f32x2{xa.BBT[0 * H + nc], xa.BBT[1 * H + nc]} : f32x2{0.f, 0.f};
    b23[i] = valid ? f32x2{xa.BBT[2 * H + nc], xa.BBT[3 * H + nc]} : f32x2{0.f, 0.f};
  }
#pragma unroll
  for (int m = 0; m < IM; ++m) uxc[m] = (m < I && lane < KX && g.foldx == 0) ? xa.UXP[(m < I ? m : 0) * KX + (lane < KX ? lane : 0)] : 0.f;

  const float* xrow = xa.x + ((size_t)rowc * g.sxB + (lane < I ? lane : 0));
  size_t xoff = 0;
  auto issue = [&](int ttarget) {
    __builtin_amdgcn_global_load_lds((gl_cvoid_t*)(xrow + xoff), (lds_void_t*)(xring + (ttarget % XW_NB) * 64), 4, 0, 0);
    if (ttarget + 1 < T) xoff += (size_t)g.sxT;
  };
  auto produce = [&](int t) {
    float sx[IM];
    const lds_f4* xr4 = (const lds_f4*)(xring + (t % XW_NB) * 64);
#pragma unroll
    for (int m4 = 0; m4 < IM / 4; ++m4) {
      const f32x4 v = xr4[m4];
      sx[4 * m4 + 0] = (rowok && 4 * m4 + 0 < I) ? v[0] : 0.f;
      sx[4 * m4 + 1] = (rowok && 4 * m4 + 1 < I) ? v[1] : 0.f;
      sx[4 * m4 + 2] = (rowok && 4 * m4 + 2 < I) ? v[2] : 0.f;
      sx[4 * m4 + 3] = (rowok && 4 * m4 + 3 < I) ? v[3] : 0.f;
    }
    float q = 0.f;
    if (g.foldx == 0) {
#pragma unroll
      for (int m = 0; m < IM; ++m) q = fmaf(sx[m], uxc[m], q);
    }
    if (g.foldx == 0 && lane < KX) qxs[(t & 1) * 32 + lane] = q;
    lds_f* dst = gxl + (size_t)(t % ring_nb) * NT * 4;
#pragma unroll
    for (int i = 0; i < XW_SLOTS; ++i) {
      if (real[i]) {
        f32x2 p01a = b01[i], p01b = f32x2{0.f, 0.f}, p23a = b23[i], p23b = f32x2{0.f, 0.f};
#pragma unroll
        for (int m = 0; m + 1 < IE; m += 2) {
          p01a = pk_fma(splat2(sx[m]), w01[i][m], p01a);
          p23a = pk_fma(splat2(sx[m]), w23[i][m], p23a);
          p01b = pk_fma(splat2(sx[m + 1]), w01[i][m + 1], p01b);
          p23b = pk_fma(splat2(sx[m + 1]), w23[i][m + 1], p23b);
        }
        if constexpr ((IE & 1) != 0) {
          p01a = pk_fma(splat2(sx[IE - 1]), w01[i][IE - 1], p01a);
          p23a = pk_fma(splat2(sx[IE - 1]), w23[i][IE - 1], p23a);
        }
        const f32x2 p01 = p01a + p01b, p23 = p23a + p23b;
        *(lds_f4*)(dst + (size_t)(lane + 64 * i) * 4) = f32x4{p01.x, p01.y, p23.x, p23.y};
      }
    }
  };
  for (int s0 = 0; s0 < XW_DIST; ++s0) issue(s0);
  asm volatile("s_waitcnt vmcnt(%0)" ::"n"(XW_DIST - 1) : "memory");
  produce(0);
  wait_vm_barrier<XW_DIST - 2>();
  for (int t = 0; t < T; ++t) {
    issue(t + XW_DIST);
    produce(t + 1);
    wait_vm_barrier<XW_DIST - 2>();
  }
}

template <int KH, int R, bool FLAT, int MAXT, int CNT, bool XW = false>
__global__ void __launch_bounds__(VG_REC_BOUNDS) rec_fwd_kernel(VGeo g, FwdArgs a, XwArgs xwargs) {
  constexpr int NP = (KH + 15) / 16, KQ = NP * 16, NC = KH / 4;
  const int tid = threadIdx.x, lane = tid & 63, wave = tid >> 6;
  const int NT = g.NT, NW = g.NW, W = g.W, H = g.H, B = g.B, T = g.T;
  const bool mover = tid >= NT;
  const bool train = a.gates != nullptr;
  const size_t sstride = (size_t)g.Bp * NT;

  extern __shared__ float4 smem4[];
  float* part = reinterpret_cast<float*>(smem4);
  float* gxs = part + 2 * R * NW * KQ;
  float* outs = gxs + FWD_NB * R * NT * 4;
  float* zero4 = outs + 2 * R * NT * 8 + 256;
  if (tid < 4) zero4[tid] = 0.f;

  if (mover) {
    constexpr int MAXS = MAXT / 64;
    constexpr int NDMA = R * MAXS;
    constexpr int DEPTH = (2 * NDMA <= 63) ? 2 : 1;
    constexpr int DIST = DEPTH + 2;
    static_assert(DIST < FWD_NB, "gx ring too shallow");
    float* spare = outs + 2 * R * NT * 8;
    int row[R];
    bool rok[R];
#pragma unroll
    for (int r = 0; r < R; ++r) {
      row[r] = blockIdx.x * R + r;
      rok[r] = row[r] < B;
    }
    if (wave == NW) {
      if constexpr (XW) {
        const __attribute__((address_space(4))) char* ka =
            (const __attribute__((address_space(4))) char*)__builtin_amdgcn_kernarg_segment_ptr();
        float* xlds = zero4 + 4;
        switch ((g.I + 3) / 4) {
          case 1: xwave_role<4>(ka, gxs, xlds, row[0], FWD_NB); break;
          case 2: xwave_role<8>(ka, gxs, xlds, row[0], FWD_NB); break;
          case 3:
            if (g.I == 9) xwave_role<12, 9>(ka, gxs, xlds, row[0], FWD_NB);
            else if (g.I == 10) xwave_role<12, 10>(ka, gxs, xlds, row[0], FWD_NB);
            else xwave_role<12>(ka, gxs, xlds, row[0], FWD_NB);
            break;
          default: xwave_role<16>(ka, gxs, xlds, row[0], FWD_NB); break;
        }
        return;
      }
      auto issue = [&](int ttarget) {
        const int tc = ttarget < T ? ttarget : T - 1;
        float* dst = gxs + (size_t)(ttarget % FWD_NB) * R * NT * 4;
#pragma unroll
        for (int r = 0; r < R; ++r)
#pragma unroll
          for (int i = 0; i < MAXS; ++i) {
            const bool real = i < NW;
            const int i0 = real ? i : 0;
            dma16(a.gx + ((size_t)tc * sstride + (size_t)row[r] * NT + lane + 64 * i0) * 4,
                  real ? dst + ((size_t)r * NT + 64 * i0) * 4 : spare);
          }
      };
      for (int s0 = 0; s0 < DIST; ++s0) issue(s0);
      wait_vm_barrier<(DIST - 2) * NDMA>();
      for (int t = 0; t < T; ++t) {
        issue(t + DIST);
        wait_vm_barrier<DEPTH * NDMA>();
      }
      return;
    }
    __builtin_amdgcn_s_setprio(3);
    if (a.prog != nullptr && lane < R && rok[lane < R ? lane : 0])
      a.prog[(size_t)(blockIdx.x * R + lane) * WR_PROG_STRIDE] = 0u;
    bool sv[R][MAXS];
    unsigned so_[R][MAXS], yo_[R][MAXS];
#pragma unroll
    for (int r = 0; r < R; ++r)
#pragma unroll
      for (int i = 0; i < MAXS; ++i) {
        const int slot = lane + 64 * (i < NW ? i : 0);
        int n;
        const bool valid = vg_slot_unit(g, slot, n);
        sv[r][i] = i < NW && valid && rok[r];
        so_[r][i] = (unsigned)(row[r] * NT + slot) * 4u;
        yo_[r][i] = (unsigned)((rok[r] ? row[r] : 0) * g.syB + n) * 4u;
      }
    constexpr int QE = 2;
    bool qv[QE];
    unsigned qsrc[QE], qdst[QE];
#pragma unroll
    for (int q = 0; q < QE; ++q) {
      const int e = lane + 64 * q;
      const int GK = g.G * KH;
      const bool in = e < R * GK;
      const int ec = in ? e : 0;
      const int r = ec / GK, jr = ec - r * GK, j = jr / KH, rr = jr - j * KH;
      const int s = (g.G == 2 && rr >= g.off1) ? 1 : 0;
      const int w0 = ((j + s) % g.G) * W;
      qv[q] = in && train && (blockIdx.x * R + r) < B;
      qsrc[q] = (unsigned)((r * NW + w0) * KQ + rr);
      qdst[q] = (unsigned)((blockIdx.x * R + r) * GK + jr);
    }
    const float* qxs = zero4 + 4 + XW_NB * 64;
    const bool qx_out = XW && train && g.foldx == 0 && rok[0] && lane < g.KX;
    constexpr bool SAFE_ST = FLAT && MAXT == 512;
    auto segment = [&](int td, int tq) {
      __builtin_amdgcn_s_setprio(3);
      const int tdc = td < 0 ? 0 : td, tqc = tq < 0 ? 0 : tq;
      const float* src = outs + (size_t)(tdc & 1) * R * NT * 8;
      const float* qsrc_ = part + (size_t)(tqc & 1) * R * NW * KQ;
      float4 g4[R][MAXS];
      float2 ch[R][MAXS];
      float v[QE][MAXS];
      float qxv = 0.f;
#pragma unroll
      for (int r = 0; r < R; ++r)
#pragma unroll
        for (int i = 0; i < MAXS; ++i) {
          const int slot = lane + 64 * (i < NW ? i : 0);
          g4[r][i] = ld4(src + ((size_t)r * NT + slot) * 4);
          ch[r][i] = *reinterpret_cast<const float2*>(src + (size_t)R * NT * 4 + ((size_t)r * NT + slot) * 2);
        }
#pragma unroll
      for (int q = 0; q < QE; ++q)
#pragma unroll
        for (int w = 0; w < MAXS; ++w) v[q][w] = qsrc_[qsrc[q] + (w < W ? w : 0) * KQ];
      if constexpr (XW) qxv = qxs[(tqc & 1) * 32 + (lane & 31)];
      __builtin_amdgcn_s_setprio(0);
      if (td >= 0) {
        char* gt = reinterpret_cast<char*>(a.gates + (size_t)td * sstride * 4);
        char* ct = reinterpret_cast<char*>(a.cs + (size_t)(td + 1) * sstride);
        char* yt = reinterpret_cast<char*>(a.y + (size_t)td * g.syT);
#pragma unroll
        for (int r = 0; r < R; ++r) {
#pragma unroll
          for (int i = 0; i < MAXS; ++i) {
            if (i < NW) {
              if (train) {
                st4_sv<SAFE_ST, !SAFE_ST>(gt, 4u * so_[r][i], g4[r][i]);
                st1_sv<SAFE_ST, !SAFE_ST>(ct, so_[r][i], ch[r][i].x);
              }
              if (sv[r][i]) st1_sv<SAFE_ST, !SAFE_ST>(yt, yo_[r][i], ch[r][i].y);
            }
          }
        }
      }
      if (tq >= 0) {
        const float* qt = a.Qs + (size_t)tq * B * g.G * KH;
#pragma unroll
        for (int q = 0; q < QE; ++q) {
          if (qv[q]) {
            float acc = 0.f;
#pragma unroll
            for (int w = 0; w < MAXS; ++w) acc += w < W ? v[q][w] : 0.f;
            st1_sv<SAFE_ST>(qt, 4u * qdst[q], acc);
          }
        }
        if constexpr (XW) {
          if (qx_out) st1_sv<SAFE_ST>(a.qxw + (size_t)tq * B * g.KX, 4u * (unsigned)(row[0] * g.KX + lane), qxv);
        }
      }
    };
    if constexpr (XW) {
      if ((a.xwave & 2) != 0) asm volatile("s_barrier" ::: "memory");
    }
    asm volatile("s_waitcnt lgkmcnt(0)\n\ts_barrier" ::: "memory");
    for (int t = 0; t < T; ++t) {
      segment(t - 1, t);
      asm volatile("s_waitcnt lgkmcnt(0)\n\ts_barrier" ::: "memory");
    }
    segment(T - 1, -1);
    return;
  }

  const int grp = tid / (64 * W);
  const int m = tid - grp * 64 * W;
  const bool valid = m < g.Hg;
  const int n = grp * g.Hg + (valid ? m : 0);

  f32x2 ve01[KH], ve23[KH], eh01, eh23;
  float ur[KQ];
  bool direct = false;
  constexpr bool CAN_DIRECT = XW && KH <= 16 && !FLAT && R == 1;
  if constexpr (CAN_DIRECT) direct = (a.xwave & 2) != 0;
  if (direct) {
    if constexpr (CAN_DIRECT) {
      float vr[4][16], ur0[16], bs[4];
#pragma unroll
      for (int k = 0; k < 4; ++k) dr_load_row<KH>(a.VE, (size_t)k * H + n, valid, vr[k]);
      dr_load_row<KH>(a.UR, (size_t)n, valid, ur0);
      {
        float bxv[4], bhv[4];
#pragma unroll
        for (int k = 0; k < 4; ++k) bxv[k] = xwargs.BBT[(size_t)k * H + n], bhv[k] = xwargs.BH[(size_t)k * H + n];
#pragma unroll
        for (int k = 0; k < 4; ++k) bs[k] = bxv[k] + bhv[k];
      }
      const float dh = a.EH[n], dxv = xwargs.DX[n < g.I ? n : 0];
      const float vf = valid ? 1.f : 0.f;
      float* wxl = zero4 + 4 + xwave_lds_floats();
      auto xside = [&](auto kxc) {
        constexpr int KX_ = decltype(kxc)::value;
        float vx[4][16];
#pragma unroll
        for (int k = 0; k < 4; ++k) dr_load_row<KX_>(xwargs.WXD, (size_t)k * H + n, valid, vx[k]);
        dr_wx_unit<KX_>(vx, bs, dxv, xwargs.UXP, g.I, NT, n, vf, tid, wxl);
      };
      if (g.KX == 16) xside(std::integral_constant<int, 16>{});
      else xside(std::integral_constant<int, 8>{});
      __builtin_amdgcn_sched_barrier(0);
#pragma unroll
      for (int rr = 0; rr < KH; ++rr) ve01[rr] = f32x2{vr[0][rr], vr[1][rr]}, ve23[rr] = f32x2{vr[2][rr], vr[3][rr]};
      eh01 = f32x2{(dh - dr_chain<KH>(ur0, vr[0])) * vf, (dh - dr_chain<KH>(ur0, vr[1])) * vf};
      eh23 = f32x2{(dh - dr_chain<KH>(ur0, vr[2])) * vf, (dh - dr_chain<KH>(ur0, vr[3])) * vf};
      float* scr = outs + (size_t)tid * DR_SCR_FLOATS;
      dr_put(scr, ur0);
      const int li = lane & 15, dn = 16 - dr_ror_dir(lane);
      sfor<16>([&](auto kk) {
        constexpr int K = decltype(kk)::value;
        ur[K] = ror16<K>(dr_at(scr, li + dn * K));
      });
      asm volatile("s_waitcnt lgkmcnt(0)\n\ts_barrier" ::: "memory");
    }
  } else {
#pragma unroll
    for (int rr = 0; rr < KH; ++rr) {
      ve01[rr] = f32x2{a.VE[(size_t)(0 * KH + rr) * NT + tid], a.VE[(size_t)(1 * KH + rr) * NT + tid]};
      ve23[rr] = f32x2{a.VE[(size_t)(2 * KH + rr) * NT + tid], a.VE[(size_t)(3 * KH + rr) * NT + tid]};
    }
    eh01 = f32x2{a.EH[0 * NT + tid], a.EH[1 * NT + tid]};
    eh23 = f32x2{a.EH[2 * NT + tid], a.EH[3 * NT + tid]};
#pragma unroll
    for (int j = 0; j < KQ; ++j) ur[j] = a.UR[(size_t)j * NT + tid];
  }

  int pb[NC];
  int pb2[FLAT ? NC : 1];
#pragma unroll
  for (int c = 0; c < NC; ++c) {
    const int s = (g.G == 2 && 4 * c >= g.off1) ? 1 : 0;
    const int q0 = FLAT ? 0 : grp;
    pb[c] = (((q0 + s) % g.G) * W) * KQ + 4 * c;
    if (FLAT) pb2[c] = (((1 + s) % g.G) * W) * KQ + 4 * c;
  }

  constexpr int NCP = NC <= 2 ? 2 : (NC <= 4 ? 4 : 8);
  constexpr bool FASTQ16 = !FLAT && NC == NCP && NC * CNT <= 16;
  constexpr bool FASTQ64 = !FLAT && !FASTQ16 && NC <= 8 && NCP * CNT <= 64;
  constexpr bool FLATQ = FLAT && NC <= 8 && NCP * CNT <= 32;
  constexpr bool FASTQ = FASTQ16 || FASTQ64 || FLATQ;
  int rdoff = 0;
  {
    const int li = FLATQ ? (lane & 31) : (FASTQ64 ? lane : (lane & 15)), cc = li % NCP, w = li / NCP;
    const int ccl = cc < NC ? cc : 0;
    const int s = (g.G == 2 && 4 * ccl >= g.off1) ? 1 : 0;
    const int q0 = FLATQ ? (lane >> 5) : grp;
    rdoff = (w < CNT && cc < NC) ? ((((q0 + s) % g.G) * W + w) * KQ + 4 * cc) : -1;
  }

  float h[R], c[R];
#pragma unroll
  for (int r = 0; r < R; ++r) {
    const int row = blockIdx.x * R + r;
    const bool ok = valid && row < B;
    const int rowc = row < B ? row : B - 1;
    h[r] = (ok && a.h0 != nullptr) ? a.h0[(size_t)rowc * H + n] : 0.f;
    c[r] = (ok && a.c0 != nullptr) ? a.c0[(size_t)rowc * H + n] : 0.f;
    if (train) a.cs[(size_t)row * NT + tid] = c[r];
  }

  for (int t = 0; t < T; ++t) {
    const int buf = t & 1;
#pragma unroll
    for (int r = 0; r < R; ++r) {
      float hv = h[r];
      dpp_fence(hv);
#pragma unroll
      for (int p = 0; p < NP; ++p) {
        float a0 = 0.f, a1 = 0.f;
        fmac_ror_x16(a0, a1, hv, &ur[p * 16]);
        const float s = rowsum4(a0 + a1);
        if (lane < 16) part[((buf * R + r) * NW + wave) * KQ + p * 16 + lane] = s;
      }
    }
    asm volatile("s_waitcnt lgkmcnt(0)\n\ts_barrier" ::: "memory");
    const float* gxt = gxs + (size_t)(t % FWD_NB) * R * NT * 4;
    float* ot = outs + (size_t)buf * R * NT * 8;
#pragma unroll
    for (int r = 0; r < R; ++r) {
      const float* src = part + (size_t)(buf * R + r) * NW * KQ;
      const float4 gx4 = ld4(gxt + ((size_t)r * NT + tid) * 4);
      float4 q[NC], q2[FLAT ? NC : 1];
      if constexpr (FASTQ) {
        const float4 v = ld4(rdoff >= 0 ? src + rdoff : zero4);
        float sx = class_sum16<NCP>(v.x), sy = class_sum16<NCP>(v.y);
        float sz = class_sum16<NCP>(v.z), sw = class_sum16<NCP>(v.w);
        if constexpr (FASTQ64) sx = rowsum4(sx), sy = rowsum4(sy), sz = rowsum4(sz), sw = rowsum4(sw);
        if constexpr (FLATQ) sx = rowsum2(sx), sy = rowsum2(sy), sz = rowsum2(sz), sw = rowsum2(sw);
#pragma unroll
        for (int cc = 0; cc < NC; ++cc)
          q[cc] = make_float4(bcast_lane(sx, cc), bcast_lane(sy, cc), bcast_lane(sz, cc), bcast_lane(sw, cc));
        if constexpr (FLATQ) {
#pragma unroll
          for (int cc = 0; cc < NC; ++cc)
            q2[cc] = make_float4(bcast_lane(sx, 32 + cc), bcast_lane(sy, 32 + cc), bcast_lane(sz, 32 + cc), bcast_lane(sw, 32 + cc));
        }
      }
#pragma unroll
      for (int cc = 0; cc < (FASTQ ? 0 : NC); ++cc) {
        float4 v[CNT];
#pragma unroll
        for (int w = 0; w < CNT; ++w) v[w] = ld4(src + pb[cc] + w * KQ);
        q[cc] = v[0];
#pragma unroll
        for (int w = 1; w < CNT; ++w) q[cc] = f4add(q[cc], v[w]);
        if (FLAT) {
#pragma unroll
          for (int w = 0; w < CNT; ++w) v[w] = ld4(src + pb2[cc] + w * KQ);
          q2[cc] = v[0];
#pragma unroll
          for (int w = 1; w < CNT; ++w) q2[cc] = f4add(q2[cc], v[w]);
        }
      }
      const f32x2 hh = splat2(h[r]);
      f32x2 p01a = pk_fma(hh, eh01, f32x2{gx4.x, gx4.y}), p01b = f32x2{0.f, 0.f};
      f32x2 p23a = pk_fma(hh, eh23, f32x2{gx4.z, gx4.w}), p23b = f32x2{0.f, 0.f};
#pragma unroll
      for (int cc = 0; cc < NC; ++cc) {
        const float4 qa = q[cc];
        const float4 qb = FLAT ? q2[cc] : q[cc];
        p01a = pk_fma(splat2(qa.x), ve01[4 * cc + 0], p01a);
        p23a = pk_fma(splat2(qb.x), ve23[4 * cc + 0], p23a);
        p01b = pk_fma(splat2(qa.y), ve01[4 * cc + 1], p01b);
        p23b = pk_fma(splat2(qb.y), ve23[4 * cc + 1], p23b);
        p01a = pk_fma(splat2(qa.z), ve01[4 * cc + 2], p01a);
        p23a = pk_fma(splat2(qb.z), ve23[4 * cc + 2], p23a);
        p01b = pk_fma(splat2(qa.w), ve01[4 * cc + 3], p01b);
        p23b = pk_fma(splat2(qb.w), ve23[4 * cc + 3], p23b);
      }
      const f32x2 pre01 = p01a + p01b, pre23 = p23a + p23b;
      const CellFwd cell = cell_fwd(pre01.x, pre01.y, pre23.x, pre23.y, c[r]);
      c[r] = cell.c, h[r] = cell.h;
      st4(ot + ((size_t)r * NT + tid) * 4, cell.gates);
      *reinterpret_cast<float2*>(ot + (size_t)R * NT * 4 + ((size_t)r * NT + tid) * 2) = make_float2(c[r], h[r]);
    }
  }
  asm volatile("s_waitcnt lgkmcnt(0)\n\ts_barrier" ::: "memory");

#pragma unroll
  for (int r = 0; r < R; ++r) {
    const int row = blockIdx.x * R + r;
    if (valid && row < B) {
      if (a.hT != nullptr) a.hT[(size_t)row * H + n] = h[r];
      if (a.cT != nullptr) a.cT[(size_t)row * H + n] = c[r];
    }
  }
  if constexpr (R == 1) {
    {
      typedef __attribute__((address_space(3))) float lds_f;
      const float* chp = outs + (size_t)((T - 1) & 1) * R * NT * 8 + (size_t)R * NT * 4;
      head_epilogue((const __attribute__((address_space(4))) char*)__builtin_amdgcn_kernarg_segment_ptr(), (const lds_f*)chp,
                    (int)blockIdx.x, wave, (lds_f*)part);
      ce_epilogue((const __attribute__((address_space(4))) char*)__builtin_amdgcn_kernarg_segment_ptr(), (int)blockIdx.x, wave, (lds_f*)part);
    }
  }
}

template <int KH, int R, bool FLAT, int MAXT, int CNT>
static int fwd_launch_one(const VGeo& g, const FwdArgs& a, const XwArgs& xw, hipStream_t s) {
  constexpr int KQ = (KH + 15) / 16 * 16;
  if (a.xwave != 0) {
    if constexpr (R == 1 && MAXT == 256 && !FLAT) {
      const size_t ldsx = sizeof(float) * ((size_t)2 * g.NW * KQ + (size_t)FWD_NB * g.NT * 4 + (size_t)2 * g.NT * 8 + 256 + 4 +
                                           xwave_lds_floats() + ((a.xwave & 2) != 0 ? (size_t)(4 * g.I + 4) * g.NT : 0));
      hipLaunchKernelGGL((rec_fwd_kernel<KH, R, FLAT, MAXT, CNT, true>), dim3(g.nwg), dim3(g.NT + 128), ldsx, s, g, a, xw);
      return (int)hipGetLastError();
    } else {
      return -3;
    }
  }
  const size_t lds = sizeof(float) * ((size_t)2 * R * g.NW * KQ + (size_t)FWD_NB * R * g.NT * 4 + (size_t)2 * R * g.NT * 8 + 256 + 4);
  auto kern = rec_fwd_kernel<KH, R, FLAT, MAXT, CNT>;
  if (lds > 64 * 1024) {
    const hipError_t e = hipFuncSetAttribute(reinterpret_cast<const void*>(kern),
                                             hipFuncAttributeMaxDynamicSharedMemorySize, (int)lds);
    if (e != hipSuccess) return (int)e;
  }
  hipLaunchKernelGGL(kern, dim3(g.nwg), dim3(g.NT + 128), lds, s, g, a, xw);
  return (int)hipGetLastError();
}

template <int KH, int MAXT, int CNT, bool ALSO_FLAT>
static int fwd_launch_mode(const VGeo& g, const FwdArgs& a, const XwArgs& xw, hipStream_t s) {
  if (g.R != 1) return -3;
  if (g.flat) {
    if constexpr (ALSO_FLAT) return g.G == 2 ? fwd_launch_one<KH, 1, true, MAXT, CNT>(g, a, xw, s) : -3;
    else return -3;
  }
  return fwd_launch_one<KH, 1, false, MAXT, CNT>(g, a, xw, s);
}

template <int KH>
static int fwd_launch_kh(const VGeo& g, const FwdArgs& a, const XwArgs& xw, hipStream_t s) {
  const int cnt = g.W;
  if (g.NT <= 256) {
    switch (cnt) {
      case 1: return fwd_launch_mode<KH, 256, 1, true>(g, a, xw, s);
      case 2: return fwd_launch_mode<KH, 256, 2, true>(g, a, xw, s);
      case 3: return fwd_launch_mode<KH, 256, 3, false>(g, a, xw, s);
      case 4: return fwd_launch_mode<KH, 256, 4, false>(g, a, xw, s);
    }
  } else if (g.NT <= 384) {
    switch (cnt) {
      case 3: return fwd_launch_mode<KH, 384, 3, true>(g, a, xw, s);
      case 5: return fwd_launch_mode<KH, 384, 5, false>(g, a, xw, s);
      case 6: return fwd_launch_mode<KH, 384, 6, false>(g, a, xw, s);
    }
  } else if (g.NT <= 512) {
    switch (cnt) {
      case 4: return fwd_launch_mode<KH, 512, 4, true>(g, a, xw, s);
      case 7: return fwd_launch_mode<KH, 512, 7, false>(g, a, xw, s);
      case 8: return fwd_launch_mode<KH, 512, 8, false>(g, a, xw, s);
    }
  }
  return -3;
}
```

vmlmf_amd/csrc/vmlmf_state.hip:

```cpp
#include <atomic>
#include <cstdlib>

#include "vmlmf_host.h"

using namespace vmlmf_host;

int vmlmf_env_switch(const char* name, EnvRule rule, int dflt) {
  const char* e = getenv(name);
  if (e == nullptr) return dflt;
  switch (rule) {
    case ENV_SET: return 1;
    case ENV_ON: return e[0] != '0';
    case ENV_INT: return atoi(e);
    case ENV_POS: break;
  }
  const int v = atoi(e);
  return v >= 1 ? v : dflt;
}

namespace vmlmf_host {

static thread_local std::string g_err = "";

int fail(int code, const std::string& msg) {
  g_err = msg;
  return code;
}

Prof g_prof;

int g_debug_sync, g_adam_guard, g_xwave, g_wchunks, g_wmin, g_rc, g_wride, g_wride_k, g_wride_maxb, g_wride_lag, g_wride_rc, g_rb_mode,
    g_rb_minB, g_rb_S, g_rb_rows, g_rec3, g_inrow, g_wring, g_direct, g_finish2, g_wf_bwd, g_pack_slim, g_finish_units, g_rbx, g_ffb;
struct Switch {
  const char* env;
  const char* key;
  int dflt;
  EnvRule rule;
  int* var;
};
const Switch g_switches[] = {
    {"VMLMF_DEBUG_SYNC", nullptr, 0, ENV_SET, &g_debug_sync},
    {"VMLMF_ADAM_GUARD", "adam_guard", 1, ENV_INT, &g_adam_guard},
    {"VMLMF_XWAVE", nullptr, 1, ENV_ON, &g_xwave},
    {"VMLMF_WCHUNKS", nullptr, 64, ENV_POS, &g_wchunks},
    {"VMLMF_WMIN", nullptr, 64, ENV_POS, &g_wmin},
    {"VMLMF_RC", nullptr, 0, ENV_POS, &g_rc},
    {"VMLMF_WRIDE", nullptr, 1, ENV_ON, &g_wride},
    {"VMLMF_WRIDE_K", nullptr, 32, ENV_POS, &g_wride_k},
    {"VMLMF_WRIDE_MAXB", nullptr, 64, ENV_POS, &g_wride_maxb},
    {"VMLMF_WRIDE_LAG", nullptr, 3, ENV_POS, &g_wride_lag},
    {"VMLMF_WRIDE_RC", nullptr, 32, ENV_POS, &g_wride_rc},
    {"VMLMF_RB", "rb", -1, ENV_INT, &g_rb_mode},
    {"VMLMF_RB_MINB", "rb_min_batch", 0, ENV_POS, &g_rb_minB},
    {"VMLMF_RB_S", "rb_cluster", 0, ENV_POS, &g_rb_S},
    {"VMLMF_RB_ROWS", "rb_rows", 0, ENV_POS, &g_rb_rows},
    {"VMLMF_REC3", "rec3", 6, ENV_INT, &g_rec3},
    {"VMLMF_INROW", "inrow", -1, ENV_INT, &g_inrow},
    {"VMLMF_WRING", "wring", -1, ENV_INT, &g_wring},
    {"VMLMF_DIRECT", "direct", 1, ENV_INT, &g_direct},
    {"VMLMF_FINISH2", "finish2", 1, ENV_INT, &g_finish2},
    {"VMLMF_WF_BWD", nullptr, 1, ENV_INT, &g_wf_bwd},
    {"VMLMF_PACK_SLIM", nullptr, 1, ENV_INT, &g_pack_slim},
    {"VMLMF_FINISH_UNITS", nullptr, 1, ENV_INT, &g_finish_units},
    {"VMLMF_RBX", "rbx", 1, ENV_INT, &g_rbx},
    {"VMLMF_FFB", "ffb", 0, ENV_INT, &g_ffb},
};
static int read_switches() {
  for (const Switch& w : g_switches) *w.var = vmlmf_env_switch(w.env, w.rule, w.dflt);
  return 0;
}
static const int g_switches_read = read_switches();
static const Switch* find_switch(const std::string& key) {
  for (const Switch& w : g_switches)
    if (w.key != nullptr && key == w.key) return &w;
  return nullptr;
}

constexpr int MAX_DEV = 16;
static std::atomic<unsigned*> g_status[MAX_DEV];
static std::atomic<bool> g_status_failed[MAX_DEV];
static std::mutex g_status_mu;
static std::atomic<unsigned*> g_health[MAX_DEV];

unsigned* status_word(hipStream_t s) {
  int dev = 0;
  if (hipGetDevice(&dev) != hipSuccess || dev < 0 || dev >= MAX_DEV) return nullptr;
  unsigned* w = g_status[dev].load(std::memory_order_acquire);
  if (w != nullptr || g_status_failed[dev].load(std::memory_order_acquire)) return w;
  std::lock_guard<std::mutex> lk(g_status_mu);
  w = g_status[dev].load(std::memory_order_acquire);
  if (w != nullptr || g_status_failed[dev].load(std::memory_order_acquire)) return w;
  hipStreamCaptureStatus cs = hipStreamCaptureStatusNone;
  if (hipStreamIsCapturing(s, &cs) != hipSuccess) { (void)hipGetLastError(); return nullptr; }
  if (cs != hipStreamCaptureStatusNone) return nullptr;
  hipStreamCaptureMode mode = hipStreamCaptureModeRelaxed;
  const bool swapped = hipThreadExchangeStreamCaptureMode(&mode) == hipSuccess;
  void* p = nullptr;
  const bool ok = hipHostMalloc(&p, 64, hipHostMallocMapped) == hipSuccess && p != nullptr;
  void* hw = nullptr;
  if (ok && hipMalloc(&hw, 256) == hipSuccess && hw != nullptr) {
    if (hipMemset(hw, 0, 256) == hipSuccess) g_health[dev].store((unsigned*)hw, std::memory_order_release);
  } else {
    (void)hipGetLastError();
  }
  if (swapped) (void)hipThreadExchangeStreamCaptureMode(&mode);
  if (ok) {
    memset(p, 0, 64);
    g_status[dev].store((unsigned*)p, std::memory_order_release);
    return (unsigned*)p;
  }
  (void)hipGetLastError();
  g_status_failed[dev].store(true, std::memory_order_release);
  return nullptr;
}
unsigned* health_word(hipStream_t s) {
  (void)status_word(s);
  int dev = 0;
  if (hipGetDevice(&dev) != hipSuccess || dev < 0 || dev >= MAX_DEV) return nullptr;
  return g_health[dev].load(std::memory_order_acquire);
}
static unsigned* status_word_if_any() {
  int dev = 0;
  if (hipGetDevice(&dev) != hipSuccess || dev < 0 || dev >= MAX_DEV) return nullptr;
  return g_status[dev].load(std::memory_order_acquire);
}

constexpr int WRIDE_SPIN_DEFAULT = 1 << 16;
int g_wride_spin = WRIDE_SPIN_DEFAULT;
std::atomic<int> g_wride_tripped{0};
std::atomic<int> g_ring_launches{0};

static const char* status_text(unsigned code) {
  switch (code) {
    case VMLMF_ST_WRIDE: return "a weight-gradient worker riding on the backward launch never saw its rows' progress words (parameter gradients of that call are NaN); the workers wait for workgroups of their own launch and need them resident: when the GPU is shared with other processes or launches that fill its CUs, run with VMLMF_WRIDE=0 (after this report the process does so by itself for eager launches)";
    case VMLMF_ST_CLUSTER: return "a member of a row-block cluster never published its partial (outputs of that call are NaN)";
    case VMLMF_ST_WF_FWD: return "a layer of a wavefront forward launch never received the rows of the layer below (outputs are NaN)";
    case VMLMF_ST_WF_BWD: return "a layer of a wavefront backward launch never received the gradient rows of the layer above (gradients are NaN)";
    case VMLMF_ST_P2P: return "a rank of the peer-to-peer all-reduce never wrote its buffer into this rank's staging area (the reduced buffer is NaN)";
  }
  return "unknown status code";
}

int g_tune_generation = 0;
int take_status() {
  unsigned* w = status_word_if_any();
  if (w == nullptr) return 0;
  const unsigned code = *(volatile unsigned*)w;
  if (code == 0) return 0;
  *(volatile unsigned*)w = 0;
  if (code == VMLMF_ST_WRIDE && g_wride_spin == WRIDE_SPIN_DEFAULT && g_wride_tripped.exchange(1) == 0) ++g_tune_generation;
  return fail(VMLMF_E_PROTOCOL, std::string("an earlier launch on this device gave up a bounded wait: ") + status_text(code));
}
int debug_status(hipStream_t s) {
  if (!g_debug_sync) return 0;
  (void)hipStreamSynchronize(s);
  return take_status();
}

static int g_cus[MAX_DEV] = {0};
int device_cus() {
  int dev = 0;
  if (hipGetDevice(&dev) != hipSuccess || dev < 0 || dev >= MAX_DEV) return 256;
  if (g_cus[dev] == 0) {
    int n = 0;
    if (hipDeviceGetAttribute(&n, hipDeviceAttributeMultiprocessorCount, dev) != hipSuccess || n <= 0) n = 256;
    g_cus[dev] = n;
  }
  return g_cus[dev];
}

int hip_fail(int rc, const char* what) {
  if (rc == 0) return 0;
  if (rc == -3) return fail(VMLMF_E_UNSUPPORTED, std::string(what) + ": no kernel instantiation for this geometry");
  return fail(rc, std::string(what) + ": " + hipGetErrorString((hipError_t)rc));
}

}

unsigned* vmlmf_health_word_if_any() {
  int dev = 0;
  if (hipGetDevice(&dev) != hipSuccess || dev < 0 || dev >= MAX_DEV) return nullptr;
  return g_health[dev].load(std::memory_order_acquire);
}
int vmlmf_adam_guard_mode() { return g_adam_guard; }

int vmlmf_set_error(int code, const std::string& msg) { return fail(code, msg); }
unsigned* vmlmf_status_word(void* stream) { return status_word((hipStream_t)stream); }

extern "C" {

int vmlmf_abi_version(void) { return VMLMF_ABI_VERSION; }

const char* vmlmf_build_info(void) { return "vmlmf_hip gfx950 fp32 persistent-rnn (register-resident U/V, DPP rank reduce)"; }

const char* vmlmf_last_error(void) { return g_err.c_str(); }

int vmlmf_tune_generation(void) { return g_tune_generation; }

int vmlmf_check_status(void) { return take_status(); }

int vmlmf_tune(const char* key, int value) {
  if (key == nullptr) return fail(VMLMF_E_BADARG, "tune: null key");
  const std::string k(key);
  const Switch* sw = find_switch(k);
  if (k == "test_wride_spin") g_wride_spin = value < 1 ? WRIDE_SPIN_DEFAULT : value;
  else if (k == "clear_health") {
    unsigned* hw = vmlmf_health_word_if_any();
    if (hw != nullptr && hipMemset(hw, 0, sizeof(unsigned)) != hipSuccess) (void)hipGetLastError();
  }
  else if (k == "wride") g_wride_tripped.store(value != 0 ? 0 : 1);
  else if (k == "rb_min_batch" || k == "rb_cluster" || k == "rb_rows") *sw->var = value < 0 ? 0 : value;
  else if (sw != nullptr) *sw->var = value;
  else return fail(VMLMF_E_BADARG, "tune: unknown key " + k);
  ++g_tune_generation;
  return 0;
}

int vmlmf_tune_get(const char* key, int* value) {
  if (key == nullptr || value == nullptr) return fail(VMLMF_E_BADARG, "tune_get: null pointer");
  const std::string k(key);
  const Switch* sw = find_switch(k);
  if (k == "wride") *value = (g_wride && g_wride_tripped.load() == 0) ? 1 : 0;
  else if (k == "wring_launches") *value = g_ring_launches.load();
  else if (sw != nullptr) *value = *sw->var;
  else return fail(VMLMF_E_BADARG, "tune_get: unknown key " + k);
  return 0;
}

int vmlmf_profile_enable(int mask) {
  std::lock_guard<std::mutex> lk(g_prof.mu);
  g_prof.mask = (unsigned)mask;
  return 0;
}

int vmlmf_profile_read(float* usec_sum, int32_t* count, int reset) {
  std::lock_guard<std::mutex> lk(g_prof.mu);
  for (int k = 0; k < NKERN; ++k) {
    float sum = 0.f;
    for (auto& pr : g_prof.ev[k]) {
      (void)hipEventSynchronize(pr.second);
      float ms = 0.f;
      (void)hipEventElapsedTime(&ms, pr.first, pr.second);
      sum += ms * 1000.f;
    }
    if (usec_sum != nullptr) usec_sum[k] = sum;
    if (count != nullptr) count[k] = (int32_t)g_prof.ev[k].size();
    if (reset) {
      for (auto& pr : g_prof.ev[k]) {
        (void)hipEventDestroy(pr.first);
        (void)hipEventDestroy(pr.second);
      }
      g_prof.ev[k].clear();
    }
  }
  return 0;
}

const char* vmlmf_kernel_name(int k) { return kernel_label(k); }

}
```

Baseline: 915,400 RNN timesteps/s.

## Spread forward recurrence output stores across three storer waves

```diff
diff --git a/vmlmf_amd/csrc/vmlmf_api.hip b/vmlmf_amd/csrc/vmlmf_api.hip
--- a/vmlmf_amd/csrc/vmlmf_api.hip
+++ b/vmlmf_amd/csrc/vmlmf_api.hip
@@ -239,6 +239,7 @@
   if (pl.family != FAM_VALU) return pl;
   const bool call = ctx == PLAN_CALL;
   if (pl.xwave && ((g_rec3 & 1) || ((g_rec3 & 4) && g.nwg > device_cus())) && rec3_fwd_supported(g)) pl.fwd = K_REC3;
+  pl.storers3 = pl.xwave && pl.fwd == K_REC && g_fwd_storers == 3 && rec_fwd_storers3_ok(g);
   const bool rec3_bwd = (g_rec3 & 2) && rec3_bwd_supported(g);
   if (call && g_inrow != 0 && !want_dx && rec4_bwd_supported(g) && (g_inrow > 0 || g.B > g_wride_maxb)) pl.bwd = K_REC4;
   else pl.bwd = rec3_bwd ? K_REC3 : K_REC;
@@ -587,6 +588,7 @@
     a.VE = p->v_h[0], a.UR = p->u_h[0], a.EH = p->dia_h, a.xwave = 3;
     xw.UXP = p->u_x, xw.WXD = p->v_x, xw.BBT = p->b_x, xw.BH = p->b_h, xw.DX = p->dia_x, xw.direct = 1;
   }
+  if (pl.storers3) a.xwave |= 4, ++g_storers3_launches;
   a.prog = g.training ? reinterpret_cast<unsigned*>(rs + L.r_prog) : nullptr;
   if ((rc = pl.fwd == K_REC3 ? run(SL_REC_FWD, s, "rec3_fwd", [&] { return launch_rec3_fwd(g, a, xw, s); })
                              : run(SL_REC_FWD, s, "rec_fwd", [&] { return launch_rec_fwd(g, a, xw, s); })) != 0) return rc;
diff --git a/vmlmf_amd/csrc/vmlmf_host.h b/vmlmf_amd/csrc/vmlmf_host.h
--- a/vmlmf_amd/csrc/vmlmf_host.h
+++ b/vmlmf_amd/csrc/vmlmf_host.h
@@ -19,10 +19,11 @@
 inline int hip_tail(int rc) { return rc == 0 ? 0 : fail(rc, hipGetErrorString((hipError_t)rc)); }
 
 extern int g_debug_sync, g_adam_guard, g_xwave, g_wchunks, g_wmin, g_rc, g_wride, g_wride_k, g_wride_maxb, g_wride_lag, g_wride_rc, g_rb_mode,
-    g_rb_minB, g_rb_S, g_rb_rows, g_rec3, g_inrow, g_wring, g_direct, g_finish2, g_wf_bwd, g_pack_slim, g_finish_units, g_rbx, g_ffb;
+    g_rb_minB, g_rb_S, g_rb_rows, g_rec3, g_inrow, g_wring, g_direct, g_finish2, g_wf_bwd, g_pack_slim, g_finish_units, g_rbx, g_ffb, g_fwd_storers;
 extern int g_wride_spin, g_tune_generation;
 extern std::atomic<int> g_wride_tripped;
 extern std::atomic<int> g_ring_launches;
+extern std::atomic<int> g_storers3_launches;
 
 enum Slot { SL_PACK, SL_XPROJ, SL_REC_FWD, SL_REC_BWD, SL_DQX_DX, SL_WGRAD, SL_REDUCE, SL_FINISH, SL_HEAD_FWD, SL_HEAD_BWD, SL_CE_FWD,
             SL_CE_BWD, SL_FINISH2, NKERN };
@@ -120,6 +121,7 @@
 struct LayerPlan {
   Family family;
   bool xwave;
+  bool storers3;
   RecKernel fwd, bwd;
   bool direct;
   bool head_inside;
diff --git a/vmlmf_amd/csrc/vmlmf_launch.h b/vmlmf_amd/csrc/vmlmf_launch.h
--- a/vmlmf_amd/csrc/vmlmf_launch.h
+++ b/vmlmf_amd/csrc/vmlmf_launch.h
@@ -172,6 +172,7 @@
 int launch_xproj(const VGeo& g, const VPack& L, const float* pack, const float* x, float* gx, float* qx,
                  hipStream_t s);
 int launch_rec_fwd(const VGeo& g, const FwdArgs& a, const XwArgs& xw, hipStream_t s);
+inline bool rec_fwd_storers3_ok(const VGeo& g) { return g.KH <= 16 && (g.W == 2 || g.W == 3); }
 int launch_rec_bwd(const VGeo& g, const BwdArgs& a, hipStream_t s);
 inline bool rec_bwd_rides(const VGeo& g) { return g.KH > 16 || g.W > 3; }
 bool rec3_fwd_supported(const VGeo& g);
diff --git a/vmlmf_amd/csrc/vmlmf_rec_fwd.inc b/vmlmf_amd/csrc/vmlmf_rec_fwd.inc
--- a/vmlmf_amd/csrc/vmlmf_rec_fwd.inc
+++ b/vmlmf_amd/csrc/vmlmf_rec_fwd.inc
@@ -256,367 +256,12 @@
 
 template <int KH, int R, bool FLAT, int MAXT, int CNT, bool XW = false>
 __global__ void __launch_bounds__(VG_REC_BOUNDS) rec_fwd_kernel(VGeo g, FwdArgs a, XwArgs xwargs) {
-  constexpr int NP = (KH + 15) / 16, KQ = NP * 16, NC = KH / 4;
-  const int tid = threadIdx.x, lane = tid & 63, wave = tid >> 6;
-  const int NT = g.NT, NW = g.NW, W = g.W, H = g.H, B = g.B, T = g.T;
-  const bool mover = tid >= NT;
-  const bool train = a.gates != nullptr;
-  const size_t sstride = (size_t)g.Bp * NT;
-
-  extern __shared__ float4 smem4[];
-  float* part = reinterpret_cast<float*>(smem4);
-  float* gxs = part + 2 * R * NW * KQ;
-  float* outs = gxs + FWD_NB * R * NT * 4;
-  float* zero4 = outs + 2 * R * NT * 8 + 256;
-  if (tid < 4) zero4[tid] = 0.f;
-
-  if (mover) {
-    constexpr int MAXS = MAXT / 64;
-    constexpr int NDMA = R * MAXS;
-    constexpr int DEPTH = (2 * NDMA <= 63) ? 2 : 1;
-    constexpr int DIST = DEPTH + 2;
-    static_assert(DIST < FWD_NB, "gx ring too shallow");
-    float* spare = outs + 2 * R * NT * 8;
-    int row[R];
-    bool rok[R];
-#pragma unroll
-    for (int r = 0; r < R; ++r) {
-      row[r] = blockIdx.x * R + r;
-      rok[r] = row[r] < B;
-    }
-    if (wave == NW) {
-      if constexpr (XW) {
-        const __attribute__((address_space(4))) char* ka =
-            (const __attribute__((address_space(4))) char*)__builtin_amdgcn_kernarg_segment_ptr();
-        float* xlds = zero4 + 4;
-        switch ((g.I + 3) / 4) {
-          case 1: xwave_role<4>(ka, gxs, xlds, row[0], FWD_NB); break;
-          case 2: xwave_role<8>(ka, gxs, xlds, row[0], FWD_NB); break;
-          case 3:
-            if (g.I == 9) xwave_role<12, 9>(ka, gxs, xlds, row[0], FWD_NB);
-            else if (g.I == 10) xwave_role<12, 10>(ka, gxs, xlds, row[0], FWD_NB);
-            else xwave_role<12>(ka, gxs, xlds, row[0], FWD_NB);
-            break;
-          default: xwave_role<16>(ka, gxs, xlds, row[0], FWD_NB); break;
-        }
-        return;
-      }
-      auto issue = [&](int ttarget) {
-        const int tc = ttarget < T ? ttarget : T - 1;
-        float* dst = gxs + (size_t)(ttarget % FWD_NB) * R * NT * 4;
-#pragma unroll
-        for (int r = 0; r < R; ++r)
-#pragma unroll
-          for (int i = 0; i < MAXS; ++i) {
-            const bool real = i < NW;
-            const int i0 = real ? i : 0;
-            dma16(a.gx + ((size_t)tc * sstride + (size_t)row[r] * NT + lane + 64 * i0) * 4,
-                  real ? dst + ((size_t)r * NT + 64 * i0) * 4 : spare);
-          }
-      };
-      for (int s0 = 0; s0 < DIST; ++s0) issue(s0);
-      wait_vm_barrier<(DIST - 2) * NDMA>();
-      for (int t = 0; t < T; ++t) {
-        issue(t + DIST);
-        wait_vm_barrier<DEPTH * NDMA>();
-      }
-      return;
-    }
-    __builtin_amdgcn_s_setprio(3);
-    if (a.prog != nullptr && lane < R && rok[lane < R ? lane : 0])
-      a.prog[(size_t)(blockIdx.x * R + lane) * WR_PROG_STRIDE] = 0u;
-    bool sv[R][MAXS];
-    unsigned so_[R][MAXS], yo_[R][MAXS];
-#pragma unroll
-    for (int r = 0; r < R; ++r)
-#pragma unroll
-      for (int i = 0; i < MAXS; ++i) {
-        const int slot = lane + 64 * (i < NW ? i : 0);
-        int n;
-        const bool valid = vg_slot_unit(g, slot, n);
-        sv[r][i] = i < NW && valid && rok[r];
-        so_[r][i] = (unsigned)(row[r] * NT + slot) * 4u;
-        yo_[r][i] = (unsigned)((rok[r] ? row[r] : 0) * g.syB + n) * 4u;
-      }
-    constexpr int QE = 2;
-    bool qv[QE];
-    unsigned qsrc[QE], qdst[QE];
-#pragma unroll
-    for (int q = 0; q < QE; ++q) {
-      const int e = lane + 64 * q;
-      const int GK = g.G * KH;
-      const bool in = e < R * GK;
-      const int ec = in ? e : 0;
-      const int r = ec / GK, jr = ec - r * GK, j = jr / KH, rr = jr - j * KH;
-      const int s = (g.G == 2 && rr >= g.off1) ? 1 : 0;
-      const int w0 = ((j + s) % g.G) * W;
-      qv[q] = in && train && (blockIdx.x * R + r) < B;
-      qsrc[q] = (unsigned)((r * NW + w0) * KQ + rr);
-      qdst[q] = (unsigned)((blockIdx.x * R + r) * GK + jr);
-    }
-    const float* qxs = zero4 + 4 + XW_NB * 64;
-    const bool qx_out = XW && train && g.foldx == 0 && rok[0] && lane < g.KX;
-    constexpr bool SAFE_ST = FLAT && MAXT == 512;
-    auto segment = [&](int td, int tq) {
-      __builtin_amdgcn_s_setprio(3);
-      const int tdc = td < 0 ? 0 : td, tqc = tq < 0 ? 0 : tq;
-      const float* src = outs + (size_t)(tdc & 1) * R * NT * 8;
-      const float* qsrc_ = part + (size_t)(tqc & 1) * R * NW * KQ;
-      float4 g4[R][MAXS];
-      float2 ch[R][MAXS];
-      float v[QE][MAXS];
-      float qxv = 0.f;
-#pragma unroll
-      for (int r = 0; r < R; ++r)
-#pragma unroll
-        for (int i = 0; i < MAXS; ++i) {
-          const int slot = lane + 64 * (i < NW ? i : 0);
-          g4[r][i] = ld4(src + ((size_t)r * NT + slot) * 4);
-          ch[r][i] = *reinterpret_cast<const float2*>(src + (size_t)R * NT * 4 + ((size_t)r * NT + slot) * 2);
-        }
-#pragma unroll
-      for (int q = 0; q < QE; ++q)
-#pragma unroll
-        for (int w = 0; w < MAXS; ++w) v[q][w] = qsrc_[qsrc[q] + (w < W ? w : 0) * KQ];
-      if constexpr (XW) qxv = qxs[(tqc & 1) * 32 + (lane & 31)];
-      __builtin_amdgcn_s_setprio(0);
-      if (td >= 0) {
-        char* gt = reinterpret_cast<char*>(a.gates + (size_t)td * sstride * 4);
-        char* ct = reinterpret_cast<char*>(a.cs + (size_t)(td + 1) * sstride);
-        char* yt = reinterpret_cast<char*>(a.y + (size_t)td * g.syT);
-#pragma unroll
-        for (int r = 0; r < R; ++r) {
-#pragma unroll
-          for (int i = 0; i < MAXS; ++i) {
-            if (i < NW) {
-              if (train) {
-                st4_sv<SAFE_ST, !SAFE_ST>(gt, 4u * so_[r][i], g4[r][i]);
-                st1_sv<SAFE_ST, !SAFE_ST>(ct, so_[r][i], ch[r][i].x);
-              }
-              if (sv[r][i]) st1_sv<SAFE_ST, !SAFE_ST>(yt, yo_[r][i], ch[r][i].y);
-            }
-          }
-        }
-      }
-      if (tq >= 0) {
-        const float* qt = a.Qs + (size_t)tq * B * g.G * KH;
-#pragma unroll
-        for (int q = 0; q < QE; ++q) {
-          if (qv[q]) {
-            float acc = 0.f;
-#pragma unroll
-            for (int w = 0; w < MAXS; ++w) acc += w < W ? v[q][w] : 0.f;
-            st1_sv<SAFE_ST>(qt, 4u * qdst[q], acc);
-          }
-        }
-        if constexpr (XW) {
-          if (qx_out) st1_sv<SAFE_ST>(a.qxw + (size_t)tq * B * g.KX, 4u * (unsigned)(row[0] * g.KX + lane), qxv);
-        }
-      }
-    };
-    if constexpr (XW) {
-      if ((a.xwave & 2) != 0) asm volatile("s_barrier" ::: "memory");
-    }
-    asm volatile("s_waitcnt lgkmcnt(0)\n\ts_barrier" ::: "memory");
-    for (int t = 0; t < T; ++t) {
-      segment(t - 1, t);
-      asm volatile("s_waitcnt lgkmcnt(0)\n\ts_barrier" ::: "memory");
-    }
-    segment(T - 1, -1);
-    return;
-  }
-
-  const int grp = tid / (64 * W);
-  const int m = tid - grp * 64 * W;
-  const bool valid = m < g.Hg;
-  const int n = grp * g.Hg + (valid ? m : 0);
-
-  f32x2 ve01[KH], ve23[KH], eh01, eh23;
-  float ur[KQ];
-  bool direct = false;
-  constexpr bool CAN_DIRECT = XW && KH <= 16 && !FLAT && R == 1;
-  if constexpr (CAN_DIRECT) direct = (a.xwave & 2) != 0;
-  if (direct) {
-    if constexpr (CAN_DIRECT) {
-      float vr[4][16], ur0[16], bs[4];
-#pragma unroll
-      for (int k = 0; k < 4; ++k) dr_load_row<KH>(a.VE, (size_t)k * H + n, valid, vr[k]);
-      dr_load_row<KH>(a.UR, (size_t)n, valid, ur0);
-      {
-        float bxv[4], bhv[4];
-#pragma unroll
-        for (int k = 0; k < 4; ++k) bxv[k] = xwargs.BBT[(size_t)k * H + n], bhv[k] = xwargs.BH[(size_t)k * H + n];
-#pragma unroll
-        for (int k = 0; k < 4; ++k) bs[k] = bxv[k] + bhv[k];
-      }
-      const float dh = a.EH[n], dxv = xwargs.DX[n < g.I ? n : 0];
-      const float vf = valid ? 1.f : 0.f;
-      float* wxl = zero4 + 4 + xwave_lds_floats();
-      auto xside = [&](auto kxc) {
-        constexpr int KX_ = decltype(kxc)::value;
-        float vx[4][16];
-#pragma unroll
-        for (int k = 0; k < 4; ++k) dr_load_row<KX_>(xwargs.WXD, (size_t)k * H + n, valid, vx[k]);
-        dr_wx_unit<KX_>(vx, bs, dxv, xwargs.UXP, g.I, NT, n, vf, tid, wxl);
-      };
-      if (g.KX == 16) xside(std::integral_constant<int, 16>{});
-      else xside(std::integral_constant<int, 8>{});
-      __builtin_amdgcn_sched_barrier(0);
-#pragma unroll
-      for (int rr = 0; rr < KH; ++rr) ve01[rr] = f32x2{vr[0][rr], vr[1][rr]}, ve23[rr] = f32x2{vr[2][rr], vr[3][rr]};
-      eh01 = f32x2{(dh - dr_chain<KH>(ur0, vr[0])) * vf, (dh - dr_chain<KH>(ur0, vr[1])) * vf};
-      eh23 = f32x2{(dh - dr_chain<KH>(ur0, vr[2])) * vf, (dh - dr_chain<KH>(ur0, vr[3])) * vf};
-      float* scr = outs + (size_t)tid * DR_SCR_FLOATS;
-      dr_put(scr, ur0);
-      const int li = lane & 15, dn = 16 - dr_ror_dir(lane);
-      sfor<16>([&](auto kk) {
-        constexpr int K = decltype(kk)::value;
-        ur[K] = ror16<K>(dr_at(scr, li + dn * K));
-      });
-      asm volatile("s_waitcnt lgkmcnt(0)\n\ts_barrier" ::: "memory");
-    }
-  } else {
-#pragma unroll
-    for (int rr = 0; rr < KH; ++rr) {
-      ve01[rr] = f32x2{a.VE[(size_t)(0 * KH + rr) * NT + tid], a.VE[(size_t)(1 * KH + rr) * NT + tid]};
-      ve23[rr] = f32x2{a.VE[(size_t)(2 * KH + rr) * NT + tid], a.VE[(size_t)(3 * KH + rr) * NT + tid]};
-    }
-    eh01 = f32x2{a.EH[0 * NT + tid], a.EH[1 * NT + tid]};
-    eh23 = f32x2{a.EH[2 * NT + tid], a.EH[3 * NT + tid]};
-#pragma unroll
-    for (int j = 0; j < KQ; ++j) ur[j] = a.UR[(size_t)j * NT + tid];
-  }
-
-  int pb[NC];
-  int pb2[FLAT ? NC : 1];
-#pragma unroll
-  for (int c = 0; c < NC; ++c) {
-    const int s = (g.G == 2 && 4 * c >= g.off1) ? 1 : 0;
-    const int q0 = FLAT ? 0 : grp;
-    pb[c] = (((q0 + s) % g.G) * W) * KQ + 4 * c;
-    if (FLAT) pb2[c] = (((1 + s) % g.G) * W) * KQ + 4 * c;
-  }
-
-  constexpr int NCP = NC <= 2 ? 2 : (NC <= 4 ? 4 : 8);
-  constexpr bool FASTQ16 = !FLAT && NC == NCP && NC * CNT <= 16;
-  constexpr bool FASTQ64 = !FLAT && !FASTQ16 && NC <= 8 && NCP * CNT <= 64;
-  constexpr bool FLATQ = FLAT && NC <= 8 && NCP * CNT <= 32;
-  constexpr bool FASTQ = FASTQ16 || FASTQ64 || FLATQ;
-  int rdoff = 0;
-  {
-    const int li = FLATQ ? (lane & 31) : (FASTQ64 ? lane : (lane & 15)), cc = li % NCP, w = li / NCP;
-    const int ccl = cc < NC ? cc : 0;
-    const int s = (g.G == 2 && 4 * ccl >= g.off1) ? 1 : 0;
-    const int q0 = FLATQ ? (lane >> 5) : grp;
-    rdoff = (w < CNT && cc < NC) ? ((((q0 + s) % g.G) * W + w) * KQ + 4 * cc) : -1;
-  }
-
-  float h[R], c[R];
-#pragma unroll
-  for (int r = 0; r < R; ++r) {
-    const int row = blockIdx.x * R + r;
-    const bool ok = valid && row < B;
-    const int rowc = row < B ? row : B - 1;
-    h[r] = (ok && a.h0 != nullptr) ? a.h0[(size_t)rowc * H + n] : 0.f;
-    c[r] = (ok && a.c0 != nullptr) ? a.c0[(size_t)rowc * H + n] : 0.f;
-    if (train) a.cs[(size_t)row * NT + tid] = c[r];
-  }
-
-  for (int t = 0; t < T; ++t) {
-    const int buf = t & 1;
-#pragma unroll
-    for (int r = 0; r < R; ++r) {
-      float hv = h[r];
-      dpp_fence(hv);
-#pragma unroll
-      for (int p = 0; p < NP; ++p) {
-        float a0 = 0.f, a1 = 0.f;
-        fmac_ror_x16(a0, a1, hv, &ur[p * 16]);
-        const float s = rowsum4(a0 + a1);
-        if (lane < 16) part[((buf * R + r) * NW + wave) * KQ + p * 16 + lane] = s;
-      }
-    }
-    asm volatile("s_waitcnt lgkmcnt(0)\n\ts_barrier" ::: "memory");
-    const float* gxt = gxs + (size_t)(t % FWD_NB) * R * NT * 4;
-    float* ot = outs + (size_t)buf * R * NT * 8;
-#pragma unroll
-    for (int r = 0; r < R; ++r) {
-      const float* src = part + (size_t)(buf * R + r) * NW * KQ;
-      const float4 gx4 = ld4(gxt + ((size_t)r * NT + tid) * 4);
-      float4 q[NC], q2[FLAT ? NC : 1];
-      if constexpr (FASTQ) {
-        const float4 v = ld4(rdoff >= 0 ? src + rdoff : zero4);
-        float sx = class_sum16<NCP>(v.x), sy = class_sum16<NCP>(v.y);
-        float sz = class_sum16<NCP>(v.z), sw = class_sum16<NCP>(v.w);
-        if constexpr (FASTQ64) sx = rowsum4(sx), sy = rowsum4(sy), sz = rowsum4(sz), sw = rowsum4(sw);
-        if constexpr (FLATQ) sx = rowsum2(sx), sy = rowsum2(sy), sz = rowsum2(sz), sw = rowsum2(sw);
-#pragma unroll
-        for (int cc = 0; cc < NC; ++cc)
-          q[cc] = make_float4(bcast_lane(sx, cc), bcast_lane(sy, cc), bcast_lane(sz, cc), bcast_lane(sw, cc));
-        if constexpr (FLATQ) {
-#pragma unroll
-          for (int cc = 0; cc < NC; ++cc)
-            q2[cc] = make_float4(bcast_lane(sx, 32 + cc), bcast_lane(sy, 32 + cc), bcast_lane(sz, 32 + cc), bcast_lane(sw, 32 + cc));
-        }
-      }
-#pragma unroll
-      for (int cc = 0; cc < (FASTQ ? 0 : NC); ++cc) {
-        float4 v[CNT];
-#pragma unroll
-        for (int w = 0; w < CNT; ++w) v[w] = ld4(src + pb[cc] + w * KQ);
-        q[cc] = v[0];
-#pragma unroll
-        for (int w = 1; w < CNT; ++w) q[cc] = f4add(q[cc], v[w]);
-        if (FLAT) {
-#pragma unroll
-          for (int w = 0; w < CNT; ++w) v[w] = ld4(src + pb2[cc] + w * KQ);
-          q2[cc] = v[0];
-#pragma unroll
-          for (int w = 1; w < CNT; ++w) q2[cc] = f4add(q2[cc], v[w]);
-        }
-      }
-      const f32x2 hh = splat2(h[r]);
-      f32x2 p01a = pk_fma(hh, eh01, f32x2{gx4.x, gx4.y}), p01b = f32x2{0.f, 0.f};
-      f32x2 p23a = pk_fma(hh, eh23, f32x2{gx4.z, gx4.w}), p23b = f32x2{0.f, 0.f};
-#pragma unroll
-      for (int cc = 0; cc < NC; ++cc) {
-        const float4 qa = q[cc];
-        const float4 qb = FLAT ? q2[cc] : q[cc];
-        p01a = pk_fma(splat2(qa.x), ve01[4 * cc + 0], p01a);
-        p23a = pk_fma(splat2(qb.x), ve23[4 * cc + 0], p23a);
-        p01b = pk_fma(splat2(qa.y), ve01[4 * cc + 1], p01b);
-        p23b = pk_fma(splat2(qb.y), ve23[4 * cc + 1], p23b);
-        p01a = pk_fma(splat2(qa.z), ve01[4 * cc + 2], p01a);
-        p23a = pk_fma(splat2(qb.z), ve23[4 * cc + 2], p23a);
-        p01b = pk_fma(splat2(qa.w), ve01[4 * cc + 3], p01b);
-        p23b = pk_fma(splat2(qb.w), ve23[4 * cc + 3], p23b);
-      }
-      const f32x2 pre01 = p01a + p01b, pre23 = p23a + p23b;
-      const CellFwd cell = cell_fwd(pre01.x, pre01.y, pre23.x, pre23.y, c[r]);
-      c[r] = cell.c, h[r] = cell.h;
-      st4(ot + ((size_t)r * NT + tid) * 4, cell.gates);
-      *reinterpret_cast<float2*>(ot + (size_t)R * NT * 4 + ((size_t)r * NT + tid) * 2) = make_float2(c[r], h[r]);
-    }
-  }
-  asm volatile("s_waitcnt lgkmcnt(0)\n\ts_barrier" ::: "memory");
-
-#pragma unroll
-  for (int r = 0; r < R; ++r) {
-    const int row = blockIdx.x * R + r;
-    if (valid && row < B) {
-      if (a.hT != nullptr) a.hT[(size_t)row * H + n] = h[r];
-      if (a.cT != nullptr) a.cT[(size_t)row * H + n] = c[r];
-    }
-  }
-  if constexpr (R == 1) {
-    {
-      typedef __attribute__((address_space(3))) float lds_f;
-      const float* chp = outs + (size_t)((T - 1) & 1) * R * NT * 8 + (size_t)R * NT * 4;
-      head_epilogue((const __attribute__((address_space(4))) char*)__builtin_amdgcn_kernarg_segment_ptr(), (const lds_f*)chp,
-                    (int)blockIdx.x, wave, (lds_f*)part);
-      ce_epilogue((const __attribute__((address_space(4))) char*)__builtin_amdgcn_kernarg_segment_ptr(), (int)blockIdx.x, wave, (lds_f*)part);
-    }
-  }
+  constexpr int NST = 1;
+#include "vmlmf_rec_fwd_body.inc"
+}
+template <int KH, int R, bool FLAT, int MAXT, int CNT, bool XW, int NST>
+__global__ void __launch_bounds__(MAXT + 64 * (NST + 1)) rec_fwd_kernel(VGeo g, FwdArgs a, XwArgs xwargs) {
+#include "vmlmf_rec_fwd_body.inc"
 }
 
 template <int KH, int R, bool FLAT, int MAXT, int CNT>
@@ -626,6 +271,12 @@
     if constexpr (R == 1 && MAXT == 256 && !FLAT) {
       const size_t ldsx = sizeof(float) * ((size_t)2 * g.NW * KQ + (size_t)FWD_NB * g.NT * 4 + (size_t)2 * g.NT * 8 + 256 + 4 +
                                            xwave_lds_floats() + ((a.xwave & 2) != 0 ? (size_t)(4 * g.I + 4) * g.NT : 0));
+      if constexpr (KH <= 16 && (CNT == 2 || CNT == 3)) {
+        if ((a.xwave & 4) != 0 && rec_fwd_storers3_ok(g)) {
+          hipLaunchKernelGGL((rec_fwd_kernel<KH, R, FLAT, MAXT, CNT, true, 3>), dim3(g.nwg), dim3(g.NT + 64 + 192), ldsx, s, g, a, xw);
+          return (int)hipGetLastError();
+        }
+      }
       hipLaunchKernelGGL((rec_fwd_kernel<KH, R, FLAT, MAXT, CNT, true>), dim3(g.nwg), dim3(g.NT + 128), ldsx, s, g, a, xw);
       return (int)hipGetLastError();
     } else {
diff --git a/vmlmf_amd/csrc/vmlmf_rec_fwd_body.inc b/vmlmf_amd/csrc/vmlmf_rec_fwd_body.inc
--- /dev/null
+++ b/vmlmf_amd/csrc/vmlmf_rec_fwd_body.inc
@@ -0,0 +1,380 @@
+  static_assert(NST == 1 || (NST == 3 && XW && R == 1 && MAXT == 256 && !FLAT), "three storers: x-projection-wave tier only");
+  constexpr int NP = (KH + 15) / 16, KQ = NP * 16, NC = KH / 4;
+  const int tid = threadIdx.x, lane = tid & 63, wave = tid >> 6;
+  const int NT = g.NT, NW = g.NW, W = g.W, H = g.H, B = g.B, T = g.T;
+  const bool mover = tid >= NT;
+  const bool train = a.gates != nullptr;
+  const size_t sstride = (size_t)g.Bp * NT;
+
+  extern __shared__ float4 smem4[];
+  float* part = reinterpret_cast<float*>(smem4);
+  float* gxs = part + 2 * R * NW * KQ;
+  float* outs = gxs + FWD_NB * R * NT * 4;
+  float* zero4 = outs + 2 * R * NT * 8 + 256;
+  if (tid < 4) zero4[tid] = 0.f;
+
+  if (mover) {
+    constexpr int MAXS = MAXT / 64;
+    constexpr int NDMA = R * MAXS;
+    constexpr int DEPTH = (2 * NDMA <= 63) ? 2 : 1;
+    constexpr int DIST = DEPTH + 2;
+    static_assert(DIST < FWD_NB, "gx ring too shallow");
+    float* spare = outs + 2 * R * NT * 8;
+    int row[R];
+    bool rok[R];
+#pragma unroll
+    for (int r = 0; r < R; ++r) {
+      row[r] = blockIdx.x * R + r;
+      rok[r] = row[r] < B;
+    }
+    if (wave == NW) {
+      if constexpr (XW) {
+        const __attribute__((address_space(4))) char* ka =
+            (const __attribute__((address_space(4))) char*)__builtin_amdgcn_kernarg_segment_ptr();
+        float* xlds = zero4 + 4;
+        switch ((g.I + 3) / 4) {
+          case 1: xwave_role<4>(ka, gxs, xlds, row[0], FWD_NB); break;
+          case 2: xwave_role<8>(ka, gxs, xlds, row[0], FWD_NB); break;
+          case 3:
+            if (g.I == 9) xwave_role<12, 9>(ka, gxs, xlds, row[0], FWD_NB);
+            else if (g.I == 10) xwave_role<12, 10>(ka, gxs, xlds, row[0], FWD_NB);
+            else xwave_role<12>(ka, gxs, xlds, row[0], FWD_NB);
+            break;
+          default: xwave_role<16>(ka, gxs, xlds, row[0], FWD_NB); break;
+        }
+        return;
+      }
+      auto issue = [&](int ttarget) {
+        const int tc = ttarget < T ? ttarget : T - 1;
+        float* dst = gxs + (size_t)(ttarget % FWD_NB) * R * NT * 4;
+#pragma unroll
+        for (int r = 0; r < R; ++r)
+#pragma unroll
+          for (int i = 0; i < MAXS; ++i) {
+            const bool real = i < NW;
+            const int i0 = real ? i : 0;
+            dma16(a.gx + ((size_t)tc * sstride + (size_t)row[r] * NT + lane + 64 * i0) * 4,
+                  real ? dst + ((size_t)r * NT + 64 * i0) * 4 : spare);
+          }
+      };
+      for (int s0 = 0; s0 < DIST; ++s0) issue(s0);
+      wait_vm_barrier<(DIST - 2) * NDMA>();
+      for (int t = 0; t < T; ++t) {
+        issue(t + DIST);
+        wait_vm_barrier<DEPTH * NDMA>();
+      }
+      return;
+    }
+    constexpr int NB = NST == 1 ? MAXS : 1;
+    const int sj = NST == 1 ? 0 : wave - NW - 1;
+    if constexpr (NST != 1) {
+      if (sj >= NW) return;
+    }
+    auto blk = [&](int i) { return NST == 1 ? (i < NW ? i : 0) : sj; };
+    auto has = [&](int i) { return NST == 1 ? i < NW : true; };
+    __builtin_amdgcn_s_setprio(3);
+    if (sj == 0 && a.prog != nullptr && lane < R && rok[lane < R ? lane : 0])
+      a.prog[(size_t)(blockIdx.x * R + lane) * WR_PROG_STRIDE] = 0u;
+    bool sv[R][NB];
+    unsigned so_[R][NB], yo_[R][NB];
+#pragma unroll
+    for (int r = 0; r < R; ++r)
+#pragma unroll
+      for (int i = 0; i < NB; ++i) {
+        const int slot = lane + 64 * blk(i);
+        int n;
+        const bool valid = vg_slot_unit(g, slot, n);
+        sv[r][i] = has(i) && valid && rok[r];
+        so_[r][i] = (unsigned)(row[r] * NT + slot) * 4u;
+        yo_[r][i] = (unsigned)((rok[r] ? row[r] : 0) * g.syB + n) * 4u;
+      }
+    constexpr int QE = 2;
+    bool qv[QE];
+    unsigned qsrc[QE], qdst[QE];
+#pragma unroll
+    for (int q = 0; q < QE; ++q) {
+      const int e = lane + 64 * q;
+      const int GK = g.G * KH;
+      const bool in = e < R * GK;
+      const int ec = in ? e : 0;
+      const int r = ec / GK, jr = ec - r * GK, j = jr / KH, rr = jr - j * KH;
+      const int s = (g.G == 2 && rr >= g.off1) ? 1 : 0;
+      const int w0 = ((j + s) % g.G) * W;
+      qv[q] = in && train && (blockIdx.x * R + r) < B;
+      qsrc[q] = (unsigned)((r * NW + w0) * KQ + rr);
+      qdst[q] = (unsigned)((blockIdx.x * R + r) * GK + jr);
+    }
+    const float* qxs = zero4 + 4 + XW_NB * 64;
+    const bool qx_out = XW && train && g.foldx == 0 && rok[0] && lane < g.KX;
+    constexpr bool SAFE_ST = FLAT && MAXT == 512;
+    auto segment = [&](int td, int tq, auto rowc) {
+      constexpr bool ROW = decltype(rowc)::value;
+      __builtin_amdgcn_s_setprio(3);
+      const int tdc = td < 0 ? 0 : td, tqc = tq < 0 ? 0 : tq;
+      const float* src = outs + (size_t)(tdc & 1) * R * NT * 8;
+      const float* qsrc_ = part + (size_t)(tqc & 1) * R * NW * KQ;
+      float4 g4[R][NB];
+      float2 ch[R][NB];
+      float v[QE][MAXS];
+      float qxv = 0.f;
+#pragma unroll
+      for (int r = 0; r < R; ++r)
+#pragma unroll
+        for (int i = 0; i < NB; ++i) {
+          const int slot = lane + 64 * blk(i);
+          g4[r][i] = ld4(src + ((size_t)r * NT + slot) * 4);
+          ch[r][i] = *reinterpret_cast<const float2*>(src + (size_t)R * NT * 4 + ((size_t)r * NT + slot) * 2);
+        }
+      if constexpr (ROW) {
+#pragma unroll
+        for (int q = 0; q < QE; ++q)
+#pragma unroll
+          for (int w = 0; w < MAXS; ++w) v[q][w] = qsrc_[qsrc[q] + (w < W ? w : 0) * KQ];
+        if constexpr (XW) qxv = qxs[(tqc & 1) * 32 + (lane & 31)];
+      }
+      __builtin_amdgcn_s_setprio(0);
+      if (td >= 0) {
+        char* gt = reinterpret_cast<char*>(a.gates + (size_t)td * sstride * 4);
+        char* ct = reinterpret_cast<char*>(a.cs + (size_t)(td + 1) * sstride);
+        char* yt = reinterpret_cast<char*>(a.y + (size_t)td * g.syT);
+#pragma unroll
+        for (int r = 0; r < R; ++r) {
+#pragma unroll
+          for (int i = 0; i < NB; ++i) {
+            if (has(i)) {
+              if (train) {
+                st4_sv<SAFE_ST, !SAFE_ST>(gt, 4u * so_[r][i], g4[r][i]);
+                st1_sv<SAFE_ST, !SAFE_ST>(ct, so_[r][i], ch[r][i].x);
+              }
+              if (sv[r][i]) st1_sv<SAFE_ST, !SAFE_ST>(yt, yo_[r][i], ch[r][i].y);
+            }
+          }
+        }
+      }
+      if constexpr (ROW) if (tq >= 0) {
+        const float* qt = a.Qs + (size_t)tq * B * g.G * KH;
+#pragma unroll
+        for (int q = 0; q < QE; ++q) {
+          if (qv[q]) {
+            float acc = 0.f;
+#pragma unroll
+            for (int w = 0; w < MAXS; ++w) acc += w < W ? v[q][w] : 0.f;
+            st1_sv<SAFE_ST>(qt, 4u * qdst[q], acc);
+          }
+        }
+        if constexpr (XW) {
+          if (qx_out) st1_sv<SAFE_ST>(a.qxw + (size_t)tq * B * g.KX, 4u * (unsigned)(row[0] * g.KX + lane), qxv);
+        }
+      }
+    };
+    if constexpr (XW) {
+      if ((a.xwave & 2) != 0) asm volatile("s_barrier" ::: "memory");
+    }
+    asm volatile("s_waitcnt lgkmcnt(0)\n\ts_barrier" ::: "memory");
+    auto drain = [&](auto rowc) {
+      for (int t = 0; t < T; ++t) {
+        segment(t - 1, t, rowc);
+        asm volatile("s_waitcnt lgkmcnt(0)\n\ts_barrier" ::: "memory");
+      }
+      segment(T - 1, -1, rowc);
+    };
+    if constexpr (NST == 1) {
+      drain(std::true_type{});
+    } else {
+      if (sj == 0) drain(std::true_type{});
+      else drain(std::false_type{});
+    }
+    return;
+  }
+
+  const int grp = tid / (64 * W);
+  const int m = tid - grp * 64 * W;
+  const bool valid = m < g.Hg;
+  const int n = grp * g.Hg + (valid ? m : 0);
+
+  f32x2 ve01[KH], ve23[KH], eh01, eh23;
+  float ur[KQ];
+  bool direct = false;
+  constexpr bool CAN_DIRECT = XW && KH <= 16 && !FLAT && R == 1;
+  if constexpr (CAN_DIRECT) direct = (a.xwave & 2) != 0;
+  if (direct) {
+    if constexpr (CAN_DIRECT) {
+      float vr[4][16], ur0[16], bs[4];
+#pragma unroll
+      for (int k = 0; k < 4; ++k) dr_load_row<KH>(a.VE, (size_t)k * H + n, valid, vr[k]);
+      dr_load_row<KH>(a.UR, (size_t)n, valid, ur0);
+      {
+        float bxv[4], bhv[4];
+#pragma unroll
+        for (int k = 0; k < 4; ++k) bxv[k] = xwargs.BBT[(size_t)k * H + n], bhv[k] = xwargs.BH[(size_t)k * H + n];
+#pragma unroll
+        for (int k = 0; k < 4; ++k) bs[k] = bxv[k] + bhv[k];
+      }
+      const float dh = a.EH[n], dxv = xwargs.DX[n < g.I ? n : 0];
+      const float vf = valid ? 1.f : 0.f;
+      float* wxl = zero4 + 4 + xwave_lds_floats();
+      auto xside = [&](auto kxc) {
+        constexpr int KX_ = decltype(kxc)::value;
+        float vx[4][16];
+#pragma unroll
+        for (int k = 0; k < 4; ++k) dr_load_row<KX_>(xwargs.WXD, (size_t)k * H + n, valid, vx[k]);
+        dr_wx_unit<KX_>(vx, bs, dxv, xwargs.UXP, g.I, NT, n, vf, tid, wxl);
+      };
+      if (g.KX == 16) xside(std::integral_constant<int, 16>{});
+      else xside(std::integral_constant<int, 8>{});
+      __builtin_amdgcn_sched_barrier(0);
+#pragma unroll
+      for (int rr = 0; rr < KH; ++rr) ve01[rr] = f32x2{vr[0][rr], vr[1][rr]}, ve23[rr] = f32x2{vr[2][rr], vr[3][rr]};
+      eh01 = f32x2{(dh - dr_chain<KH>(ur0, vr[0])) * vf, (dh - dr_chain<KH>(ur0, vr[1])) * vf};
+      eh23 = f32x2{(dh - dr_chain<KH>(ur0, vr[2])) * vf, (dh - dr_chain<KH>(ur0, vr[3])) * vf};
+      float* scr = outs + (size_t)tid * DR_SCR_FLOATS;
+      dr_put(scr, ur0);
+      const int li = lane & 15, dn = 16 - dr_ror_dir(lane);
+      sfor<16>([&](auto kk) {
+        constexpr int K = decltype(kk)::value;
+        ur[K] = ror16<K>(dr_at(scr, li + dn * K));
+      });
+      asm volatile("s_waitcnt lgkmcnt(0)\n\ts_barrier" ::: "memory");
+    }
+  } else {
+#pragma unroll
+    for (int rr = 0; rr < KH; ++rr) {
+      ve01[rr] = f32x2{a.VE[(size_t)(0 * KH + rr) * NT + tid], a.VE[(size_t)(1 * KH + rr) * NT + tid]};
+      ve23[rr] = f32x2{a.VE[(size_t)(2 * KH + rr) * NT + tid], a.VE[(size_t)(3 * KH + rr) * NT + tid]};
+    }
+    eh01 = f32x2{a.EH[0 * NT + tid], a.EH[1 * NT + tid]};
+    eh23 = f32x2{a.EH[2 * NT + tid], a.EH[3 * NT + tid]};
+#pragma unroll
+    for (int j = 0; j < KQ; ++j) ur[j] = a.UR[(size_t)j * NT + tid];
+  }
+
+  int pb[NC];
+  int pb2[FLAT ? NC : 1];
+#pragma unroll
+  for (int c = 0; c < NC; ++c) {
+    const int s = (g.G == 2 && 4 * c >= g.off1) ? 1 : 0;
+    const int q0 = FLAT ? 0 : grp;
+    pb[c] = (((q0 + s) % g.G) * W) * KQ + 4 * c;
+    if (FLAT) pb2[c] = (((1 + s) % g.G) * W) * KQ + 4 * c;
+  }
+
+  constexpr int NCP = NC <= 2 ? 2 : (NC <= 4 ? 4 : 8);
+  constexpr bool FASTQ16 = !FLAT && NC == NCP && NC * CNT <= 16;
+  constexpr bool FASTQ64 = !FLAT && !FASTQ16 && NC <= 8 && NCP * CNT <= 64;
+  constexpr bool FLATQ = FLAT && NC <= 8 && NCP * CNT <= 32;
+  constexpr bool FASTQ = FASTQ16 || FASTQ64 || FLATQ;
+  int rdoff = 0;
+  {
+    const int li = FLATQ ? (lane & 31) : (FASTQ64 ? lane : (lane & 15)), cc = li % NCP, w = li / NCP;
+    const int ccl = cc < NC ? cc : 0;
+    const int s = (g.G == 2 && 4 * ccl >= g.off1) ? 1 : 0;
+    const int q0 = FLATQ ? (lane >> 5) : grp;
+    rdoff = (w < CNT && cc < NC) ? ((((q0 + s) % g.G) * W + w) * KQ + 4 * cc) : -1;
+  }
+
+  float h[R], c[R];
+#pragma unroll
+  for (int r = 0; r < R; ++r) {
+    const int row = blockIdx.x * R + r;
+    const bool ok = valid && row < B;
+    const int rowc = row < B ? row : B - 1;
+    h[r] = (ok && a.h0 != nullptr) ? a.h0[(size_t)rowc * H + n] : 0.f;
+    c[r] = (ok && a.c0 != nullptr) ? a.c0[(size_t)rowc * H + n] : 0.f;
+    if (train) a.cs[(size_t)row * NT + tid] = c[r];
+  }
+
+  for (int t = 0; t < T; ++t) {
+    const int buf = t & 1;
+#pragma unroll
+    for (int r = 0; r < R; ++r) {
+      float hv = h[r];
+      dpp_fence(hv);
+#pragma unroll
+      for (int p = 0; p < NP; ++p) {
+        float a0 = 0.f, a1 = 0.f;
+        fmac_ror_x16(a0, a1, hv, &ur[p * 16]);
+        const float s = rowsum4(a0 + a1);
+        if (lane < 16) part[((buf * R + r) * NW + wave) * KQ + p * 16 + lane] = s;
+      }
+    }
+    asm volatile("s_waitcnt lgkmcnt(0)\n\ts_barrier" ::: "memory");
+    const float* gxt = gxs + (size_t)(t % FWD_NB) * R * NT * 4;
+    float* ot = outs + (size_t)buf * R * NT * 8;
+#pragma unroll
+    for (int r = 0; r < R; ++r) {
+      const float* src = part + (size_t)(buf * R + r) * NW * KQ;
+      const float4 gx4 = ld4(gxt + ((size_t)r * NT + tid) * 4);
+      float4 q[NC], q2[FLAT ? NC : 1];
+      if constexpr (FASTQ) {
+        const float4 v = ld4(rdoff >= 0 ? src + rdoff : zero4);
+        float sx = class_sum16<NCP>(v.x), sy = class_sum16<NCP>(v.y);
+        float sz = class_sum16<NCP>(v.z), sw = class_sum16<NCP>(v.w);
+        if constexpr (FASTQ64) sx = rowsum4(sx), sy = rowsum4(sy), sz = rowsum4(sz), sw = rowsum4(sw);
+        if constexpr (FLATQ) sx = rowsum2(sx), sy = rowsum2(sy), sz = rowsum2(sz), sw = rowsum2(sw);
+#pragma unroll
+        for (int cc = 0; cc < NC; ++cc)
+          q[cc] = make_float4(bcast_lane(sx, cc), bcast_lane(sy, cc), bcast_lane(sz, cc), bcast_lane(sw, cc));
+        if constexpr (FLATQ) {
+#pragma unroll
+          for (int cc = 0; cc < NC; ++cc)
+            q2[cc] = make_float4(bcast_lane(sx, 32 + cc), bcast_lane(sy, 32 + cc), bcast_lane(sz, 32 + cc), bcast_lane(sw, 32 + cc));
+        }
+      }
+#pragma unroll
+      for (int cc = 0; cc < (FASTQ ? 0 : NC); ++cc) {
+        float4 v[CNT];
+#pragma unroll
+        for (int w = 0; w < CNT; ++w) v[w] = ld4(src + pb[cc] + w * KQ);
+        q[cc] = v[0];
+#pragma unroll
+        for (int w = 1; w < CNT; ++w) q[cc] = f4add(q[cc], v[w]);
+        if (FLAT) {
+#pragma unroll
+          for (int w = 0; w < CNT; ++w) v[w] = ld4(src + pb2[cc] + w * KQ);
+          q2[cc] = v[0];
+#pragma unroll
+          for (int w = 1; w < CNT; ++w) q2[cc] = f4add(q2[cc], v[w]);
+        }
+      }
+      const f32x2 hh = splat2(h[r]);
+      f32x2 p01a = pk_fma(hh, eh01, f32x2{gx4.x, gx4.y}), p01b = f32x2{0.f, 0.f};
+      f32x2 p23a = pk_fma(hh, eh23, f32x2{gx4.z, gx4.w}), p23b = f32x2{0.f, 0.f};
+#pragma unroll
+      for (int cc = 0; cc < NC; ++cc) {
+        const float4 qa = q[cc];
+        const float4 qb = FLAT ? q2[cc] : q[cc];
+        p01a = pk_fma(splat2(qa.x), ve01[4 * cc + 0], p01a);
+        p23a = pk_fma(splat2(qb.x), ve23[4 * cc + 0], p23a);
+        p01b = pk_fma(splat2(qa.y), ve01[4 * cc + 1], p01b);
+        p23b = pk_fma(splat2(qb.y), ve23[4 * cc + 1], p23b);
+        p01a = pk_fma(splat2(qa.z), ve01[4 * cc + 2], p01a);
+        p23a = pk_fma(splat2(qb.z), ve23[4 * cc + 2], p23a);
+        p01b = pk_fma(splat2(qa.w), ve01[4 * cc + 3], p01b);
+        p23b = pk_fma(splat2(qb.w), ve23[4 * cc + 3], p23b);
+      }
+      const f32x2 pre01 = p01a + p01b, pre23 = p23a + p23b;
+      const CellFwd cell = cell_fwd(pre01.x, pre01.y, pre23.x, pre23.y, c[r]);
+      c[r] = cell.c, h[r] = cell.h;
+      st4(ot + ((size_t)r * NT + tid) * 4, cell.gates);
+      *reinterpret_cast<float2*>(ot + (size_t)R * NT * 4 + ((size_t)r * NT + tid) * 2) = make_float2(c[r], h[r]);
+    }
+  }
+  asm volatile("s_waitcnt lgkmcnt(0)\n\ts_barrier" ::: "memory");
+
+#pragma unroll
+  for (int r = 0; r < R; ++r) {
+    const int row = blockIdx.x * R + r;
+    if (valid && row < B) {
+      if (a.hT != nullptr) a.hT[(size_t)row * H + n] = h[r];
+      if (a.cT != nullptr) a.cT[(size_t)row * H + n] = c[r];
+    }
+  }
+  if constexpr (R == 1) {
+    {
+      typedef __attribute__((address_space(3))) float lds_f;
+      const float* chp = outs + (size_t)((T - 1) & 1) * R * NT * 8 + (size_t)R * NT * 4;
+      head_epilogue((const __attribute__((address_space(4))) char*)__builtin_amdgcn_kernarg_segment_ptr(), (const lds_f*)chp,
+                    (int)blockIdx.x, wave, (lds_f*)part);
+      ce_epilogue((const __attribute__((address_space(4))) char*)__builtin_amdgcn_kernarg_segment_ptr(), (int)blockIdx.x, wave, (lds_f*)part);
+    }
+  }
diff --git a/vmlmf_amd/csrc/vmlmf_state.hip b/vmlmf_amd/csrc/vmlmf_state.hip
--- a/vmlmf_amd/csrc/vmlmf_state.hip
+++ b/vmlmf_amd/csrc/vmlmf_state.hip
@@ -30,7 +30,7 @@
 Prof g_prof;
 
 int g_debug_sync, g_adam_guard, g_xwave, g_wchunks, g_wmin, g_rc, g_wride, g_wride_k, g_wride_maxb, g_wride_lag, g_wride_rc, g_rb_mode,
-    g_rb_minB, g_rb_S, g_rb_rows, g_rec3, g_inrow, g_wring, g_direct, g_finish2, g_wf_bwd, g_pack_slim, g_finish_units, g_rbx, g_ffb;
+    g_rb_minB, g_rb_S, g_rb_rows, g_rec3, g_inrow, g_wring, g_direct, g_finish2, g_wf_bwd, g_pack_slim, g_finish_units, g_rbx, g_ffb, g_fwd_storers;
 struct Switch {
   const char* env;
   const char* key;
@@ -64,6 +64,7 @@
     {"VMLMF_FINISH_UNITS", nullptr, 1, ENV_INT, &g_finish_units},
     {"VMLMF_RBX", "rbx", 1, ENV_INT, &g_rbx},
     {"VMLMF_FFB", "ffb", 0, ENV_INT, &g_ffb},
+    {"VMLMF_FWD_STORERS", "fwd_storers", 3, ENV_INT, &g_fwd_storers},
 };
 static int read_switches() {
   for (const Switch& w : g_switches) *w.var = vmlmf_env_switch(w.env, w.rule, w.dflt);
@@ -129,6 +130,7 @@
 int g_wride_spin = WRIDE_SPIN_DEFAULT;
 std::atomic<int> g_wride_tripped{0};
 std::atomic<int> g_ring_launches{0};
+std::atomic<int> g_storers3_launches{0};
 
 static const char* status_text(unsigned code) {
   switch (code) {
@@ -222,6 +224,7 @@
   const Switch* sw = find_switch(k);
   if (k == "wride") *value = (g_wride && g_wride_tripped.load() == 0) ? 1 : 0;
   else if (k == "wring_launches") *value = g_ring_launches.load();
+  else if (k == "fwd_storers3_launches") *value = g_storers3_launches.load();
   else if (sw != nullptr) *value = *sw->var;
   else return fail(VMLMF_E_BADARG, "tune_get: unknown key " + k);
   return 0;
```

Result: no change. 920,500 RNN timesteps/s (median of 6 runs) (+0.6%).
